# samyak0210/ViNet

Hardware: AMD Instinct MI355X
Metric: clips/sec training (32x224x384 bf16) (higher is better)
Workload: dtype bf16; 1 GPU; ViNet DHF1K training, 32x224x384 bf16, 192 clip(s)/GPU/step, kldiv + fused Adam, 1xMI355X; global_batch=192, local_batch=192, parallelism=dp1

## Files before the change

### include/vinet_hip.h

```cpp
#ifndef VINET_HIP_H
#define VINET_HIP_H

#include <stddef.h>
#include <stdint.h>

#ifdef __cplusplus
extern "C" {
#endif

#define VINET_ABI_VERSION 16

enum { VINET_F32 = 0, VINET_BF16 = 1,
       VINET_F32S = 2 };
enum { VINET_ACT_NONE = 0, VINET_ACT_RELU = 1, VINET_ACT_SIGMOID = 2 };
enum { VINET_CONV_GENERIC = 0, VINET_CONV_STEM = 1 };

typedef struct VinetTensor {
  void* ptr;
  int32_t B, T, H, W, C;
  int32_t ld;
  int64_t sB;
} VinetTensor;

typedef struct VinetAffine {
  const float* scale;
  const float* shift;
  int32_t relu;
} VinetAffine;

typedef struct VinetConvDesc {
  int32_t dtype;
  int32_t out_dtype;
  int32_t mode;
  VinetTensor x;
  VinetTensor y;
  int32_t oT, oH, oW;
  int32_t sT, sH, sW;
  int32_t omT, omH, omW, ooT, ooH, ooW;
  int32_t ntaps;
  const int32_t* taps;
  const void* w;
  int32_t Kp;
  VinetAffine pre;
  const float* out_scale;
  const float* out_shift;
  int32_t act;
  int32_t accumulate;
  float* stats;
  int32_t n_valid;
  float* splitk_ws;
  int64_t splitk_ws_bytes;
  int32_t tline;
  int32_t tpad;
  const void* bnb_z;
  int32_t bnb_ld;
  int64_t bnb_sB;
  VinetAffine bnb_fwd;
  const float* bnb_mean;
  const float* bnb_invstd;
  float* bnb_partials;
} VinetConvDesc;

int vinet_conv3d(const VinetConvDesc* desc, void* stream);
int64_t vinet_conv3d_splitk_bytes(const VinetConvDesc* desc);
int vinet_conv3d_fuses_dgrad_phases(const VinetConvDesc* desc);
int vinet_conv3d_bn_bwd_stats_rows(const VinetConvDesc* desc);
int vinet_conv3d_applies_pre_once(const VinetConvDesc* desc);
int vinet_conv3d_tile_m(const VinetConvDesc* desc);
int vinet_conv3d_stats_rows(const VinetConvDesc* desc);
int vinet_conv3d_kernel_name(const VinetConvDesc* desc, char* buf, int32_t n);

typedef struct VinetWgradDesc {
  int32_t dtype;
  int32_t mode;
  VinetTensor x;
  VinetTensor dy;
  int32_t sT, sH, sW;
  int32_t ntaps;
  const int32_t* taps;
  float* dw;
  int32_t Kp;
  VinetAffine pre;
  int32_t tline;
  int32_t tpad;
  const void* bnb_z;
  int32_t bnb_ld;
  int64_t bnb_sB;
  VinetAffine bnb_fwd;
  const float* bnb_mean;
  const float* bnb_invstd;
  const float* bnb_c1;
  const float* bnb_c2;
  int32_t max_cus;
} VinetWgradDesc;

int vinet_conv3d_wgrad(const VinetWgradDesc* desc, void* stream);
int vinet_conv3d_wgrad_fuses_bn_bwd(const VinetWgradDesc* desc);
int vinet_conv3d_wgrad_kernel_name(const VinetWgradDesc* desc, char* buf, int32_t n);

int vinet_pack_weights(const float* w, int32_t N, int32_t Cin, int32_t ntaps, int32_t transpose, int32_t stem,
                       int32_t dtype, void* out, void* stream);

int vinet_pack_weights_multi(const int64_t* table, int32_t njobs, int64_t total, int32_t dtype, void* stream);
int vinet_unpack_wgrad(float* dw, int32_t N, int32_t Cin, int32_t ntaps, int32_t stem, int32_t flags,
                       float* grad, void* stream);
int vinet_unpack_wgrad_multi(const int64_t* table, int32_t njobs, int64_t total, int32_t flags, void* stream);

int vinet_import_ncdhw(const float* src, int64_t sb, int64_t sc, int64_t st, int64_t sh, int64_t sw, int32_t C,
                       const VinetTensor* dst, int32_t dst_dtype, void* stream);
int vinet_import_ncdhw_pad(const float* src, int64_t sb, int64_t sc, int64_t st, int64_t sh, int64_t sw, int32_t C,
                           int32_t Hs, int32_t Ws, int32_t pad_top, int32_t pad_left, const VinetTensor* dst,
                           int32_t dst_dtype, void* stream);
int vinet_export_ncdhw(const VinetTensor* src, int32_t src_dtype, VinetAffine pre, float* dst, int64_t sb, int64_t sc,
                       int64_t st, int64_t sh, int64_t sw, int32_t accumulate, void* stream);
int vinet_copy_affine(const VinetTensor* src, int32_t src_dtype, VinetAffine pre, const VinetTensor* dst,
                      int32_t dst_dtype, int32_t accumulate, void* stream);

int vinet_bn_finalize(const float* partials, int32_t rows, int32_t C, int32_t ld, double count, const float* gamma,
                      const float* beta, float eps, float momentum, float* running_mean, float* running_var,
                      float* mean, float* invstd, float* scale, float* shift, void* stream);
int vinet_bn_partials_fold(const float* partials, int32_t rows, int32_t C, float* out, int32_t out_rows, void* stream);
int vinet_bn_fold(const float* gamma, const float* beta, const float* running_mean, const float* running_var,
                  const float* conv_bias , float eps, int32_t C, float* scale, float* shift,
                  float* invstd , void* stream);
int vinet_channel_stats(const VinetTensor* x, int32_t dtype, float* partials, void* stream);
int vinet_stats_rows(const VinetTensor* x);
int vinet_bn_bwd_reduce(const VinetTensor* dz, const VinetTensor* x_raw, int32_t dtype, VinetAffine fwd,
                        const float* mean, const float* invstd, float* partials, void* stream);
int vinet_bn_bwd_finalize(const float* partials, int32_t rows, int32_t C, int32_t ld, double count, const float* scale,
                          int32_t train, float* dgamma_acc, float* dbeta_acc, const float* invstd, float* c1, float* c2,
                          void* stream);
int vinet_bn_bwd_apply(const VinetTensor* dz, const VinetTensor* x_raw, int32_t dtype, VinetAffine fwd,
                       const float* mean, const float* invstd, const float* c1, const float* c2,
                       const VinetTensor* dx, void* stream);
int vinet_bn_bwd_apply_split(const VinetTensor* dz, const VinetTensor* x_raw, VinetAffine fwd, const float* mean,
                             const float* invstd, const float* c1, const float* c2, const VinetTensor* dx,
                             const VinetTensor* hi, const VinetTensor* lo, void* stream);
int vinet_act_bwd(const VinetTensor* dz, int32_t dz_dtype, const VinetTensor* z, int32_t z_dtype, int32_t act,
                  const VinetTensor* dy, int32_t dy_dtype, void* stream);
int vinet_channel_sum(const VinetTensor* x, int32_t dtype, float* workspace, int32_t Cout, float* out,
                      int32_t accumulate, void* stream);

typedef struct VinetPoolDesc {
  int32_t dtype;
  int32_t kT, kH, kW, sT, sH, sW, pT, pH, pW;
} VinetPoolDesc;
int vinet_maxpool3d(const VinetPoolDesc* d, const VinetTensor* x, VinetAffine pre, const VinetTensor* y,
                    uint8_t* argmax, void* stream);
int vinet_maxpool3d_bwd(const VinetPoolDesc* d, const VinetTensor* dy, const uint8_t* argmax, const VinetTensor* dx,
                        int32_t accumulate, void* stream);
int vinet_maxpool3d_kernel_name(const VinetPoolDesc* d, const VinetTensor* x, VinetAffine pre, const VinetTensor* y,
                                const uint8_t* argmax, char* buf, int32_t n);
int vinet_maxpool3d_bwd_kernel_name(const VinetPoolDesc* d, const VinetTensor* dy, const uint8_t* argmax,
                                    const VinetTensor* dx, char* buf, int32_t n);

int vinet_upsample2x(const VinetTensor* x, const VinetTensor* y, int32_t dtype, void* stream);
int vinet_upsample2x_bwd(const VinetTensor* dy, const VinetTensor* dx, int32_t dtype, int32_t accumulate, void* stream);
int vinet_upsample2x_bwd_relu(const VinetTensor* dy, const VinetTensor* dx, const VinetTensor* xf, int32_t dtype, void* stream);

int vinet_unfold1d(const VinetTensor* x, const VinetTensor* y, int32_t dtype, int32_t stride, int32_t pad, void* stream);

int vinet_loss_fwd(int32_t which, const float* s, const void* gt, int32_t gt_is_f64, int32_t B, int32_t n,
                   double* saved, float* loss, void* stream);
int vinet_loss_bwd(int32_t which, const float* s, const void* gt, int32_t gt_is_f64, int32_t B, int32_t n,
                   const double* saved, const float* gscale, float coeff, int32_t accumulate, float* ds, void* stream);

size_t vinet_auc_judd_workspace(int32_t B, int32_t n);
int vinet_auc_judd(const void* s, int32_t s_is_f64, const void* fix, int32_t fix_is_f64, int32_t B, int32_t n,
                   int32_t fp_offset, void* workspace, size_t workspace_bytes, double* score, int32_t* nfix,
                   int32_t* above, void* stream);

size_t vinet_auc_shuffled_workspace(int32_t B, int32_t n, int32_t nsplits, double step);
int vinet_auc_shuffled(const void* s, int32_t s_is_f64, const void* fix, int32_t fix_is_f64, const void* other,
                       int32_t other_kind, int64_t other_stride, int32_t B, int32_t n, int32_t nsplits, double step,
                       int64_t seed, const int64_t* frame_ids, const int32_t* samples, int32_t kmax, void* workspace,
                       size_t workspace_bytes, double* score, int32_t* nfix, int32_t* nother, int32_t* samples_out,
                       void* stream);

size_t vinet_auc_borji_workspace(int32_t B, int32_t n, int32_t nsplits, double step);
int vinet_auc_borji(const void* s, int32_t s_is_f64, const void* fix, int32_t fix_is_f64, int32_t B, int32_t n, int32_t nsplits,
                    double step, int64_t seed, const int64_t* frame_ids, const int32_t* samples, int32_t kmax, void* workspace,
                    size_t workspace_bytes, double* score, int32_t* nfix, int32_t* samples_out, void* stream);

int vinet_info_gain(const void* s, int32_t s_is_f64, const void* fix, int32_t fix_is_f64, const void* baseline,
                    int32_t baseline_is_f64, int64_t baseline_stride, int32_t B, int32_t n, double* score, int32_t* nfix,
                    void* stream);

size_t vinet_emd_workspace(int32_t B, int32_t R, int32_t C);
int vinet_emd(const void* s, int32_t s_is_f64, int32_t Hs, int32_t Ws, const void* gt, int32_t gt_is_f64, int32_t Hg, int32_t Wg,
              int32_t B, int32_t downsize, int32_t R, int32_t C, const double* w_gt_r, const double* w_gt_c, const double* w_s_r,
              const double* w_s_c, void* workspace, size_t workspace_bytes, double* score, int64_t* cost, int32_t* status,
              double* hist_out, void* stream);
int vinet_emd_hist(const double* P, const double* Q, int32_t B, int32_t R, int32_t C, void* workspace, size_t workspace_bytes,
                   double* score, int64_t* cost, int32_t* status, void* stream);

int vinet_adam_step(float* p, const float* g, float* m, float* v, int64_t n, float lr, float beta1, float beta2,
                    float eps, float bias_c1, float bias_c2, float grad_scale, void* stream);

int vinet_bilinear_fwd(const void* x1, const void* x2, int32_t dtype, const float* w, const float* bias, int32_t B,
                       int32_t C, int32_t I, int32_t J, int32_t O, void* out, void* stream);
int vinet_bilinear_bwd(const void* x1, const void* x2, const void* dout, int32_t dtype, const float* w, int32_t B,
                       int32_t C, int32_t I, int32_t J, int32_t O, void* dx1, void* dx2, float* dw, float* dbias,
                       void* stream);

typedef struct VinetTransformerDesc {
  int32_t dtype;
  int32_t B, S, E, H, F, L;
  int32_t train;
  float p, eps;
  uint64_t seed;
  int64_t* step;
  const float* pe;
  const void* const* params;
  void* const* grads;
  void* ws;
  int64_t ws_bytes;
  uint8_t* masks;
} VinetTransformerDesc;
int64_t vinet_transformer_workspace(const VinetTransformerDesc* desc);
int vinet_transformer_fwd(const VinetTransformerDesc* desc, const VinetTensor* x, const VinetTensor* y, void* stream);
int vinet_transformer_bwd(const VinetTransformerDesc* desc, const VinetTensor* dy, const VinetTensor* dx, void* stream);

typedef struct VinetTokenEncoderDesc {
  int32_t dtype;
  int32_t B, S, E, H, F, L;
  int32_t train;
  float p, eps;
  uint64_t seed;
  int64_t* step;
  const float* pe;
  const void* const* params;
  void* const* grads;
  void* ws;
  int64_t ws_bytes;
  uint8_t* masks;
} VinetTokenEncoderDesc;
int64_t vinet_token_encoder_workspace(const VinetTokenEncoderDesc* desc);
int vinet_token_encoder_fwd(const VinetTokenEncoderDesc* desc, const VinetTensor* x, const VinetTensor* y, void* stream);
int vinet_token_encoder_bwd(const VinetTokenEncoderDesc* desc, const VinetTensor* dy, const VinetTensor* dx, void* stream);
int vinet_token_split_fwd(const VinetTensor* x, int32_t dtype, int32_t n_audio, const VinetTensor* y, void* stream);
int vinet_token_split_bwd(const VinetTensor* dy, int32_t dtype, int32_t n_audio, const VinetTensor* dx, void* stream);

int vinet_resize_blur(const float* src, int32_t B, int32_t H, int32_t W, float* dst, int32_t oH, int32_t oW,
                      uint32_t* minmax, void* stream);
int vinet_minmax(const float* src, int32_t B, int64_t n, uint32_t* minmax, void* stream);
int vinet_normalize_u8(const float* src, const uint32_t* minmax, int32_t B, int64_t n, uint8_t* dst, void* stream);

int64_t vinet_frames_preprocess_ws_bytes(int32_t N, int32_t H, int32_t W, int32_t oH, int32_t oW);
int vinet_frames_preprocess(const uint8_t* src, int32_t N, int32_t H, int32_t W, float* dst, int32_t oH, int32_t oW,
                            const float* mean_std, void* ws, void* stream);
int vinet_audio_excerpt(const float* wav, int64_t n_samples, int64_t start, int64_t end, float* out, int32_t win, void* stream);
int64_t vinet_gt_preprocess_ws_bytes(int32_t N, int32_t oH, int32_t oW);
int vinet_gt_preprocess(const uint8_t* src, int32_t N, int32_t H, int32_t W, float* dst, int32_t oH, int32_t oW, void* ws,
                        void* stream);

int vinet_set_option(const char* name, int32_t value);
int vinet_split_bf16(const VinetTensor* src, VinetAffine pre, const VinetTensor* hi, const VinetTensor* lo, void* stream);
int vinet_fill_f32(float* p, int64_t n, float value, void* stream);
int vinet_debug_spin(int64_t cycles, void* stream);
int vinet_abi_version(void);
const char* vinet_last_error(void);

#ifdef __cplusplus
}
#endif
#endif
```

### vinet_amd/_lib.py

```python
import ctypes as C
import os

HERE = os.path.dirname(os.path.abspath(__file__))
LIB_PATH = os.environ.get("VINET_LIB") or os.path.join(HERE, "libvinet_hip.so")

F32, BF16 = 0, 1
F32S = 2
ACT_NONE, ACT_RELU, ACT_SIGMOID = 0, 1, 2
CONV_GENERIC, CONV_STEM = 0, 1
ABI_VERSION = 16


class CTensor(C.Structure):
    _fields_ = [("ptr", C.c_void_p), ("B", C.c_int32), ("T", C.c_int32), ("H", C.c_int32), ("W", C.c_int32),
                ("C", C.c_int32), ("ld", C.c_int32), ("sB", C.c_int64)]


class CAffine(C.Structure):
    _fields_ = [("scale", C.c_void_p), ("shift", C.c_void_p), ("relu", C.c_int32)]


class CConvDesc(C.Structure):
    _fields_ = [("dtype", C.c_int32), ("out_dtype", C.c_int32), ("mode", C.c_int32), ("x", CTensor), ("y", CTensor),
                ("oT", C.c_int32), ("oH", C.c_int32), ("oW", C.c_int32),
                ("sT", C.c_int32), ("sH", C.c_int32), ("sW", C.c_int32),
                ("omT", C.c_int32), ("omH", C.c_int32), ("omW", C.c_int32),
                ("ooT", C.c_int32), ("ooH", C.c_int32), ("ooW", C.c_int32),
                ("ntaps", C.c_int32), ("taps", C.c_void_p), ("w", C.c_void_p), ("Kp", C.c_int32),
                ("pre", CAffine), ("out_scale", C.c_void_p), ("out_shift", C.c_void_p),
                ("act", C.c_int32), ("accumulate", C.c_int32), ("stats", C.c_void_p), ("n_valid", C.c_int32),
                ("splitk_ws", C.c_void_p), ("splitk_ws_bytes", C.c_int64), ("tline", C.c_int32), ("tpad", C.c_int32),
                ("bnb_z", C.c_void_p), ("bnb_ld", C.c_int32), ("bnb_sB", C.c_int64), ("bnb_fwd", CAffine),
                ("bnb_mean", C.c_void_p), ("bnb_invstd", C.c_void_p), ("bnb_partials", C.c_void_p)]


class CWgradDesc(C.Structure):
    _fields_ = [("dtype", C.c_int32), ("mode", C.c_int32), ("x", CTensor), ("dy", CTensor),
                ("sT", C.c_int32), ("sH", C.c_int32), ("sW", C.c_int32),
                ("ntaps", C.c_int32), ("taps", C.c_void_p), ("dw", C.c_void_p), ("Kp", C.c_int32), ("pre", CAffine),
                ("tline", C.c_int32), ("tpad", C.c_int32),
                ("bnb_z", C.c_void_p), ("bnb_ld", C.c_int32), ("bnb_sB", C.c_int64), ("bnb_fwd", CAffine),
                ("bnb_mean", C.c_void_p), ("bnb_invstd", C.c_void_p), ("bnb_c1", C.c_void_p), ("bnb_c2", C.c_void_p),
                ("max_cus", C.c_int32)]


class CPoolDesc(C.Structure):
    _fields_ = [("dtype", C.c_int32)] + [(n, C.c_int32) for n in ("kT", "kH", "kW", "sT", "sH", "sW", "pT", "pH", "pW")]


class CTransformerDesc(C.Structure):
    _fields_ = [("dtype", C.c_int32), ("B", C.c_int32), ("S", C.c_int32), ("E", C.c_int32), ("H", C.c_int32), ("F", C.c_int32),
                ("L", C.c_int32), ("train", C.c_int32), ("p", C.c_float), ("eps", C.c_float), ("seed", C.c_uint64),
                ("step", C.c_void_p), ("pe", C.c_void_p), ("params", C.POINTER(C.c_void_p)), ("grads", C.POINTER(C.c_void_p)),
                ("ws", C.c_void_p), ("ws_bytes", C.c_int64), ("masks", C.c_void_p)]


class CTokenEncoderDesc(C.Structure):
    _fields_ = list(CTransformerDesc._fields_)


_vp, _i32, _i64, _f32, _f64 = C.c_void_p, C.c_int32, C.c_int64, C.c_float, C.c_double
_PT, _PC, _PW, _PP = C.POINTER(CTensor), C.POINTER(CConvDesc), C.POINTER(CWgradDesc), C.POINTER(CPoolDesc)
_PX = C.POINTER(CTransformerDesc)
_PK = C.POINTER(CTokenEncoderDesc)

SIGNATURES = {
    "vinet_conv3d": [_PC, _vp],
    "vinet_conv3d_tile_m": [_PC],
    "vinet_conv3d_stats_rows": [_PC],
    "vinet_conv3d_applies_pre_once": [_PC],
    "vinet_conv3d_splitk_bytes": [_PC],
    "vinet_conv3d_kernel_name": [_PC, C.c_char_p, _i32],
    "vinet_conv3d_wgrad": [_PW, _vp],
    "vinet_conv3d_wgrad_kernel_name": [_PW, C.c_char_p, _i32],
    "vinet_pack_weights": [_vp, _i32, _i32, _i32, _i32, _i32, _i32, _vp, _vp],
    "vinet_unpack_wgrad": [_vp, _i32, _i32, _i32, _i32, _i32, _vp, _vp],
    "vinet_import_ncdhw": [_vp, _i64, _i64, _i64, _i64, _i64, _i32, _PT, _i32, _vp],
    "vinet_import_ncdhw_pad": [_vp, _i64, _i64, _i64, _i64, _i64, _i32, _i32, _i32, _i32, _i32, _PT, _i32, _vp],
    "vinet_export_ncdhw": [_PT, _i32, CAffine, _vp, _i64, _i64, _i64, _i64, _i64, _i32, _vp],
    "vinet_copy_affine": [_PT, _i32, CAffine, _PT, _i32, _i32, _vp],
    "vinet_bn_finalize": [_vp, _i32, _i32, _i32, _f64, _vp, _vp, _f32, _f32, _vp, _vp, _vp, _vp, _vp, _vp, _vp],
    "vinet_bn_fold": [_vp, _vp, _vp, _vp, _vp, _f32, _i32, _vp, _vp, _vp, _vp],
    "vinet_channel_stats": [_PT, _i32, _vp, _vp],
    "vinet_stats_rows": [_PT],
    "vinet_bn_bwd_reduce": [_PT, _PT, _i32, CAffine, _vp, _vp, _vp, _vp],
    "vinet_conv3d_wgrad_fuses_bn_bwd": [_PW],
    "vinet_conv3d_fuses_dgrad_phases": [_PC],
    "vinet_conv3d_bn_bwd_stats_rows": [_PC],
    "vinet_bn_partials_fold": [_vp, _i32, _i32, _vp, _i32, _vp],
    "vinet_bn_bwd_finalize": [_vp, _i32, _i32, _i32, _f64, _vp, _i32, _vp, _vp, _vp, _vp, _vp, _vp],
    "vinet_bn_bwd_apply": [_PT, _PT, _i32, CAffine, _vp, _vp, _vp, _vp, _PT, _vp],
    "vinet_bn_bwd_apply_split": [_PT, _PT, CAffine, _vp, _vp, _vp, _vp, _PT, _PT, _PT, _vp],
    "vinet_act_bwd": [_PT, _i32, _PT, _i32, _i32, _PT, _i32, _vp],
    "vinet_channel_sum": [_PT, _i32, _vp, _i32, _vp, _i32, _vp],
    "vinet_maxpool3d": [_PP, _PT, CAffine, _PT, _vp, _vp],
    "vinet_maxpool3d_bwd": [_PP, _PT, _vp, _PT, _i32, _vp],
    "vinet_maxpool3d_kernel_name": [_PP, _PT, CAffine, _PT, _vp, C.c_char_p, _i32],
    "vinet_maxpool3d_bwd_kernel_name": [_PP, _PT, _vp, _PT, C.c_char_p, _i32],
    "vinet_upsample2x": [_PT, _PT, _i32, _vp],
    "vinet_unfold1d": [_PT, _PT, _i32, _i32, _i32, _vp],
    "vinet_upsample2x_bwd": [_PT, _PT, _i32, _i32, _vp],
    "vinet_upsample2x_bwd_relu": [_PT, _PT, _PT, _i32, _vp],
    "vinet_loss_fwd": [_i32, _vp, _vp, _i32, _i32, _i32, _vp, _vp, _vp],
    "vinet_loss_bwd": [_i32, _vp, _vp, _i32, _i32, _i32, _vp, _vp, _f32, _i32, _vp, _vp],
    "vinet_auc_judd_workspace": [_i32, _i32],
    "vinet_auc_judd": [_vp, _i32, _vp, _i32, _i32, _i32, _i32, _vp, C.c_size_t, _vp, _vp, _vp, _vp],
    "vinet_auc_shuffled_workspace": [_i32, _i32, _i32, _f64],
    "vinet_auc_shuffled": [_vp, _i32, _vp, _i32, _vp, _i32, _i64, _i32, _i32, _i32, _f64, _i64, _vp, _vp, _i32, _vp, C.c_size_t,
                           _vp, _vp, _vp, _vp, _vp],
    "vinet_auc_borji_workspace": [_i32, _i32, _i32, _f64],
    "vinet_auc_borji": [_vp, _i32, _vp, _i32, _i32, _i32, _i32, _f64, _i64, _vp, _vp, _i32, _vp, C.c_size_t, _vp, _vp, _vp, _vp],
    "vinet_info_gain": [_vp, _i32, _vp, _i32, _vp, _i32, _i64, _i32, _i32, _vp, _vp, _vp],
    "vinet_emd_workspace": [_i32, _i32, _i32],
    "vinet_emd": [_vp, _i32, _i32, _i32, _vp, _i32, _i32, _i32, _i32, _i32, _i32, _i32, _vp, _vp, _vp, _vp, _vp, C.c_size_t, _vp, _vp, _vp, _vp,
                  _vp],
    "vinet_emd_hist": [_vp, _vp, _i32, _i32, _i32, _vp, C.c_size_t, _vp, _vp, _vp, _vp],
    "vinet_adam_step": [_vp, _vp, _vp, _vp, _i64, _f32, _f32, _f32, _f32, _f32, _f32, _f32, _vp],
    "vinet_bilinear_fwd": [_vp, _vp, _i32, _vp, _vp, _i32, _i32, _i32, _i32, _i32, _vp, _vp],
    "vinet_bilinear_bwd": [_vp, _vp, _vp, _i32, _vp, _i32, _i32, _i32, _i32, _i32, _vp, _vp, _vp, _vp, _vp],
    "vinet_transformer_workspace": [_PX],
    "vinet_transformer_fwd": [_PX, _PT, _PT, _vp],
    "vinet_transformer_bwd": [_PX, _PT, _PT, _vp],
    "vinet_token_encoder_workspace": [_PK],
    "vinet_token_encoder_fwd": [_PK, _PT, _PT, _vp],
    "vinet_token_encoder_bwd": [_PK, _PT, _PT, _vp],
    "vinet_token_split_fwd": [_PT, _i32, _i32, _PT, _vp],
    "vinet_token_split_bwd": [_PT, _i32, _i32, _PT, _vp],
    "vinet_resize_blur": [_vp, _i32, _i32, _i32, _vp, _i32, _i32, _vp, _vp],
    "vinet_minmax": [_vp, _i32, _i64, _vp, _vp],
    "vinet_normalize_u8": [_vp, _vp, _i32, _i64, _vp, _vp],
    "vinet_frames_preprocess_ws_bytes": [_i32, _i32, _i32, _i32, _i32],
    "vinet_frames_preprocess": [_vp, _i32, _i32, _i32, _vp, _i32, _i32, C.POINTER(C.c_float), _vp, _vp],
    "vinet_audio_excerpt": [_vp, _i64, _i64, _i64, _vp, _i32, _vp],
    "vinet_gt_preprocess_ws_bytes": [_i32, _i32, _i32],
    "vinet_gt_preprocess": [_vp, _i32, _i32, _i32, _vp, _i32, _i32, _vp, _vp],
    "vinet_set_option": [C.c_char_p, _i32],
    "vinet_pack_weights_multi": [_vp, _i32, _i64, _i32, _vp],
    "vinet_unpack_wgrad_multi": [_vp, _i32, _i64, _i32, _vp],
    "vinet_fill_f32": [_vp, _i64, _f32, _vp],
    "vinet_split_bf16": [_PT, CAffine, _PT, _PT, _vp],
    "vinet_debug_spin": [_i64, _vp],
    "vinet_abi_version": [],
    "vinet_last_error": [],
}
_RESTYPE = {"vinet_last_error": C.c_char_p, "vinet_conv3d_splitk_bytes": C.c_int64, "vinet_frames_preprocess_ws_bytes": C.c_int64,
            "vinet_gt_preprocess_ws_bytes": C.c_int64, "vinet_auc_judd_workspace": C.c_size_t, "vinet_auc_shuffled_workspace": C.c_size_t, "vinet_auc_borji_workspace": C.c_size_t,
            "vinet_emd_workspace": C.c_size_t,
            "vinet_transformer_workspace": C.c_int64, "vinet_token_encoder_workspace": C.c_int64}

_LIB = None
_TEST_DOUBLE = None


class VinetLibraryError(RuntimeError):
    pass


def load(path=LIB_PATH):
    global _LIB
    if _LIB is not None:
        return _LIB
    if not os.path.exists(path):
        raise VinetLibraryError(
            "libvinet_hip.so is missing (%s). Build it with `python -m vinet_amd.build` "
            "(hipcc --offload-arch=gfx950); there is no CPU fallback." % path)
    import torch
    lib = C.CDLL(path)
    for name, argtypes in SIGNATURES.items():
        try:
            fn = getattr(lib, name)
        except AttributeError:
            raise VinetLibraryError("libvinet_hip.so does not export %s" % name)
        fn.argtypes = argtypes
        fn.restype = _RESTYPE.get(name, C.c_int)
    if lib.vinet_abi_version() != ABI_VERSION:
        raise VinetLibraryError("libvinet_hip.so ABI %d != expected %d" % (lib.vinet_abi_version(), ABI_VERSION))
    _LIB = lib
    return lib


LIB_OPTIONS = {}


def set_option(name, value):
    lib = get()
    rc = lib.vinet_set_option(name.encode() if isinstance(name, str) else name, int(value))
    if rc != 0:
        msg = lib.vinet_last_error()
        raise VinetLibraryError("set_option(%s): %s" % (name, msg.decode() if isinstance(msg, bytes) else msg))
    LIB_OPTIONS[name if isinstance(name, str) else name.decode()] = int(value)


def get():
    if _TEST_DOUBLE is not None:
        return _TEST_DOUBLE
    return load()


def is_test_double():
    return _TEST_DOUBLE is not None


def _install_test_double(obj):
    global _TEST_DOUBLE
    _TEST_DOUBLE = obj


def check(rc, what=""):
    if rc != 0:
        lib = get()
        msg = lib.vinet_last_error()
        if isinstance(msg, bytes):
            msg = msg.decode()
        raise RuntimeError("libvinet_hip %s failed (rc=%d): %s" % (what, rc, msg))
```

### vinet_amd/build.py

```python
import os
import subprocess
import sys
from concurrent.futures import ThreadPoolExecutor

HERE = os.path.dirname(os.path.abspath(__file__))
ROOT = os.path.dirname(HERE)
CSRC = os.path.join(HERE, "csrc")
OBJ = os.path.join(CSRC, "obj")
LIB = os.path.join(HERE, "libvinet_hip.so")
SOURCES = ["conv_api.hip", "conv_bf16.hip", "conv_bnb.hip", "conv_f32.hip", "conv_wgrad.hip", "wgrad_dma.hip", "wgrad_pp.hip", "wgrad_ts.hip", "conv_ts.hip", "wgrad_hs.hip", "wgrad_rs.hip", "wgrad_tf.hip", "conv_hs.hip", "layout.hip", "bn.hip", "pool.hip", "resample.hip", "loss_adam.hip", "metrics.hip", "emd.hip", "postproc.hip", "preproc.hip", "transformer.hip", "token_encoder.hip"]
import glob
HEADERS = sorted(glob.glob(os.path.join(CSRC, "*.h"))) + sorted(glob.glob(os.path.join(ROOT, "include", "*.h")))
FLAGS = ["--offload-arch=gfx950", "-O3", "-std=c++17", "-fPIC", "-I" + os.path.join(ROOT, "include"), "-I" + CSRC,
         "-Wno-unused-result", "-ffp-contract=off"]


GUARDED = {"conv_bf16.hip": ("conv_pw_kernel",), "pool.hip": ("maxpool_bwd",), "conv_bnb.hip": ()}
RESOURCES = os.path.join(CSRC, "obj", "kernel_resources.json")


def _parse_resources(text):
    import re
    out, cur = {}, None
    keys = {"VGPRs": "vgpr", "AGPRs": "agpr", "TotalSGPRs": "sgpr", "ScratchSize [bytes/lane]": "scratch", "VGPRs Spill": "vgpr_spill",
            "SGPRs Spill": "sgpr_spill", "Occupancy [waves/SIMD]": "occupancy"}
    for line in text.splitlines():
        m = re.search(r"remark:\s+Function Name: (\S+)", line)
        if m:
            cur = out.setdefault(m.group(1), {})
            continue
        m = re.search(r"remark:\s+([A-Za-z \[\]/]+): (\d+)", line)
        if m and cur is not None and m.group(1).strip() in keys:
            cur[keys[m.group(1).strip()]] = int(m.group(2))
    return out


def check_guarded(src, text):
    res = _parse_resources(text)
    bad = [(k, v) for k, v in res.items() if any(g in k for g in GUARDED.get(src, ())) and v.get("vgpr_spill", 0) > 0]
    if bad:
        raise RuntimeError("vector-register spills in kernels whose inline asm owns in-flight registers (%s): %s" % (src, bad))
    return res


def _hipcc():
    for c in (os.environ.get("HIPCC"), "/opt/rocm/bin/hipcc", "hipcc"):
        if c and (os.path.isabs(c) and os.path.exists(c) or not os.path.isabs(c)):
            return c
    raise RuntimeError("hipcc not found")


def _stale(target, deps):
    if not os.path.exists(target):
        return True
    t = os.path.getmtime(target)
    return any(os.path.getmtime(d) > t for d in deps)


def build_variant(tag, extra_flags, verbose=True):
    global OBJ, LIB, FLAGS
    save = (OBJ, LIB, FLAGS)
    OBJ, LIB, FLAGS = os.path.join(CSRC, "obj_" + tag), os.path.join(HERE, "libvinet_hip_%s.so" % tag), FLAGS + list(extra_flags)
    try:
        return build(force=False, verbose=verbose)
    finally:
        OBJ, LIB, FLAGS = save


def build(force=False, verbose=True):
    os.makedirs(OBJ, exist_ok=True)
    hipcc = _hipcc()
    hdrs = [h if os.path.isabs(h) else os.path.join(CSRC, h) for h in HEADERS]
    jobs = []
    for src in SOURCES:
        s = os.path.join(CSRC, src)
        o = os.path.join(OBJ, src.replace(".hip", ".o"))
        if force or _stale(o, [s] + hdrs):
            jobs.append((s, o))

    def compile_one(job):
        s, o = job
        guarded = os.path.basename(s) in GUARDED
        cmd = [hipcc] + FLAGS + (["-Rpass-analysis=kernel-resource-usage"] if guarded else []) + ["-c", s, "-o", o]
        r = subprocess.run(cmd, capture_output=True, text=True)
        out = r.stdout + r.stderr
        if guarded and r.returncode == 0:
            try:
                res = check_guarded(os.path.basename(s), out)
            except RuntimeError:
                os.remove(o)
                raise
            out = "\n".join(l for l in out.splitlines() if "kernel-resource-usage" not in l and not l.startswith("   ") )
            return s, r.returncode, out, res
        return s, r.returncode, out, None

    if jobs:
        if verbose:
            print("[vinet_amd.build] compiling %d file(s) for gfx950 ..." % len(jobs), flush=True)
        with ThreadPoolExecutor(max_workers=min(len(jobs), os.cpu_count() or 4)) as ex:
            resources, failed = {}, None
            for s, rc, out, res in ex.map(compile_one, jobs):
                if rc != 0:
                    failed = failed or RuntimeError("hipcc failed on %s:\n%s" % (s, out))
                    continue
                if res is not None:
                    resources[os.path.basename(s)] = res
                if verbose and out.strip():
                    print(out)
        if resources:
            import json
            try:
                allres = json.load(open(RESOURCES)) if os.path.exists(RESOURCES) else {}
            except ValueError:
                allres = {}
            allres.update(resources)
            with open(RESOURCES, "w") as f:
                json.dump(allres, f, indent=1, sort_keys=True)
        if failed is not None:
            raise failed
    objs = [os.path.join(OBJ, s.replace(".hip", ".o")) for s in SOURCES]
    if force or jobs or _stale(LIB, objs):
        cmd = [hipcc, "--offload-arch=gfx950", "-shared", "-fPIC", "-o", LIB] + objs
        r = subprocess.run(cmd, capture_output=True, text=True)
        if r.returncode != 0:
            raise RuntimeError("link failed:\n" + r.stdout + r.stderr)
        if verbose:
            print("[vinet_amd.build] linked", LIB, flush=True)
        try:
            audit_packed_fp32(LIB, verbose)
        except RuntimeError:
            os.remove(LIB)
            raise
    return LIB


def audit_packed_fp32(lib, verbose=True):
    import importlib.util
    spec = importlib.util.spec_from_file_location("vinet_isa_audit", os.path.join(ROOT, "tools", "isa_audit.py"))
    ia = importlib.util.module_from_spec(spec)
    spec.loader.exec_module(ia)
    if not os.path.exists(ia.OBJDUMP):
        print("[vinet_amd.build] WARNING: %s missing -- the packed-fp32 erratum audit of %s did NOT run" % (ia.OBJDUMP, lib), file=sys.stderr, flush=True)
        return None
    hits = ia.packed_fp32_high_half_reads(lib)
    if hits:
        raise RuntimeError("packed fp32 instructions with op_sel:[x,1] (MI355X erratum form) in %s: %s -- build those kernels with VN_NO_PK_F32" % (lib, hits))
    if verbose:
        print("[vinet_amd.build] packed-fp32 erratum audit: clean", flush=True)
    return hits


if __name__ == "__main__":
    build(force="--force" in sys.argv)
```

### vinet_amd/csrc/bn.hip

```cpp
#include "elementwise.h"

__global__ void bn_finalize_kernel(const float* __restrict__ partials, int rows, int C, int ld, double count,
                                   const float* gamma, const float* beta, float eps, float momentum,
                                   float* running_mean, float* running_var, float* mean_o, float* invstd_o,
                                   float* scale_o, float* shift_o) {
  const int c = blockIdx.x;
  double s = 0.0, q = 0.0;
  for (int r = threadIdx.x; r < rows; r += blockDim.x) {
    s += (double)partials[((long)r * 2 + 0) * ld + c];
    q += (double)partials[((long)r * 2 + 1) * ld + c];
  }
  __shared__ double red[2][4];
  s = wave_sum_d(s); q = wave_sum_d(q);
  if ((threadIdx.x & 63) == 0) { red[0][threadIdx.x >> 6] = s; red[1][threadIdx.x >> 6] = q; }
  __syncthreads();
  if (threadIdx.x == 0) {
    s = red[0][0] + red[0][1] + red[0][2] + red[0][3];
    q = red[1][0] + red[1][1] + red[1][2] + red[1][3];
    const double mean = s / count;
    double var = q / count - mean * mean;
    if (var < 0.0) var = 0.0;
    const double invstd = 1.0 / sqrt(var + (double)eps);
    const float g = gamma ? gamma[c] : 1.f, b = beta ? beta[c] : 0.f;
    const float sc = (float)(g * invstd);
    if (mean_o) mean_o[c] = (float)mean;
    if (invstd_o) invstd_o[c] = (float)invstd;
    scale_o[c] = sc;
    shift_o[c] = b - (float)mean * sc;
    if (running_mean) running_mean[c] = (1.f - momentum) * running_mean[c] + momentum * (float)mean;
    if (running_var) {
      const double unbiased = count > 1.0 ? var * count / (count - 1.0) : var;
      running_var[c] = (1.f - momentum) * running_var[c] + momentum * (float)unbiased;
    }
  }
}

extern "C" int vinet_bn_finalize(const float* partials, int32_t rows, int32_t C, int32_t ld, double count, const float* gamma,
                                 const float* beta, float eps, float momentum, float* running_mean, float* running_var,
                                 float* mean, float* invstd, float* scale, float* shift, void* stream) {
  VN_CHECK_ARG(partials && rows > 0 && C > 0 && (ld == 0 || ld >= C) && count > 0 && scale && shift, "bn_finalize: bad arguments");
  hipLaunchKernelGGL(bn_finalize_kernel, dim3(C), dim3(256), 0, (hipStream_t)stream, partials, rows, C, ld ? ld : C, count, gamma,
                     beta, eps, momentum, running_mean, running_var, mean, invstd, scale, shift);
  return vn_launch_status("bn_finalize");
}

__global__ __launch_bounds__(256) void bn_partials_fold_kernel(const float* __restrict__ partials, int rows, int C, int per,
                                                               float* __restrict__ out) {
  const int c = blockIdx.y * 64 + (threadIdx.x & 63), rl = threadIdx.x >> 6;
  const int r0 = blockIdx.x * per;
  int r1 = r0 + per; if (r1 > rows) r1 = rows;
  double s = 0.0, q = 0.0;
  if (c < C) {
    int r = r0 + rl;
    for (; r + 28 < r1; r += 32) {
      float a[8], b[8];
#pragma unroll
      for (int u = 0; u < 8; ++u) {
        a[u] = partials[((long)(r + 4 * u) * 2 + 0) * C + c];
        b[u] = partials[((long)(r + 4 * u) * 2 + 1) * C + c];
      }
#pragma unroll
      for (int u = 0; u < 8; ++u) { s += (double)a[u]; q += (double)b[u]; }
    }
    for (; r < r1; r += 4) {
      s += (double)partials[((long)r * 2 + 0) * C + c];
      q += (double)partials[((long)r * 2 + 1) * C + c];
    }
  }
  __shared__ double red[2][4][64];
  red[0][rl][threadIdx.x & 63] = s; red[1][rl][threadIdx.x & 63] = q;
  __syncthreads();
  if (rl == 0 && c < C) {
    const int l = threadIdx.x;
    out[((long)blockIdx.x * 2 + 0) * C + c] = (float)(red[0][0][l] + red[0][1][l] + red[0][2][l] + red[0][3][l]);
    out[((long)blockIdx.x * 2 + 1) * C + c] = (float)(red[1][0][l] + red[1][1][l] + red[1][2][l] + red[1][3][l]);
  }
}

extern "C" int vinet_bn_partials_fold(const float* partials, int32_t rows, int32_t C, float* out, int32_t out_rows, void* stream) {
  VN_CHECK_ARG(partials && out && rows > 0 && C > 0 && out_rows > 0 && out_rows <= rows, "bn_partials_fold: bad arguments");
  const int per = (rows + out_rows - 1) / out_rows;
  VN_CHECK_ARG((long)(out_rows - 1) * per < rows, "bn_partials_fold: out_rows=%d leaves empty chunks for rows=%d", out_rows, rows);
  hipLaunchKernelGGL(bn_partials_fold_kernel, dim3(out_rows, (C + 63) / 64), dim3(256), 0, (hipStream_t)stream, partials, rows, C, per, out);
  return vn_launch_status("bn_partials_fold");
}

__global__ void bn_fold_kernel(const float* gamma, const float* beta, const float* rm, const float* rv,
                               const float* conv_bias, float eps, int C, float* scale, float* shift, float* invstd) {
  const int c = blockIdx.x * blockDim.x + threadIdx.x;
  if (c >= C) return;
  const float is = 1.f / sqrtf(rv[c] + eps);
  const float sc = (gamma ? gamma[c] : 1.f) * is;
  scale[c] = sc;
  shift[c] = (beta ? beta[c] : 0.f) + ((conv_bias ? conv_bias[c] : 0.f) - rm[c]) * sc;
  if (invstd) invstd[c] = is;
}

extern "C" int vinet_bn_fold(const float* gamma, const float* beta, const float* running_mean,
                             const float* running_var, const float* conv_bias, float eps, int32_t C, float* scale,
                             float* shift, float* invstd, void* stream) {
  VN_CHECK_ARG(running_mean && running_var && scale && shift && C > 0, "bn_fold: bad arguments");
  hipLaunchKernelGGL(bn_fold_kernel, dim3((C + 255) / 256), dim3(256), 0, (hipStream_t)stream, gamma, beta,
                     running_mean, running_var, conv_bias, eps, C, scale, shift, invstd);
  return vn_launch_status("bn_fold");
}


template <typename T, int MODE>
__global__ __launch_bounds__(256) VN_NO_PK_F32 void channel_reduce8_kernel(TView x, TView dz, Affine fwd, const float* mean,
                                                              const float* invstd, long nvox, long vb,
                                                              float* __restrict__ partials) {
  const int G = x.C / 8;
  const int Gb = G < 256 ? G : 256;
  const int R = 256 / Gb;
  const int r = threadIdx.x / Gb;
  const int g0 = threadIdx.x % Gb;
  __shared__ float red[256 * 16];
  constexpr int U = 4;
  const long v0 = vb ? (long)blockIdx.x * vb : (long)blockIdx.x * R * U;
  long v1 = vb ? v0 + vb : nvox; if (v1 > nvox) v1 = nvox;
  const long vstep = vb ? (long)R * U : (long)gridDim.x * R * U;
  for (int g = g0; g < G; g += Gb) {
    float s[8], p[8], mu[8], is[8], sc[8], sh[8];
#pragma unroll
    for (int e = 0; e < 8; ++e) { s[e] = 0.f; p[e] = 0.f; mu[e] = 0.f; is[e] = 1.f; sc[e] = 1.f; sh[e] = 0.f; }
    if (r < R) {
      if (MODE == 1) {
#pragma unroll
        for (int e = 0; e < 8; ++e) { mu[e] = mean[g * 8 + e]; is[e] = invstd[g * 8 + e]; }
        if (fwd.relu) {
#pragma unroll
          for (int e = 0; e < 8; ++e) { sc[e] = fwd.scale ? fwd.scale[g * 8 + e] : 1.f; sh[e] = fwd.shift ? fwd.shift[g * 8 + e] : 0.f; }
        }
      }
      for (long vq = v0 + r; vq < v1; vq += vstep) {
        float xv[U][8], gv[U][8];
        bool ok[U];
#pragma unroll
        for (int u = 0; u < U; ++u) {
          const long v = vq + (long)u * R;
          ok[u] = v < v1;
          if (ok[u]) {
            if (MODE == 1) {
              ld8_nt<T>((const T*)x.p + vox_lin(x, v) + g * 8, xv[u]);
              ld8_nt<T>((const T*)dz.p + vox_lin(dz, v) + g * 8, gv[u]);
            } else {
              ld8<T>((const T*)x.p + vox_lin(x, v) + g * 8, xv[u]);
            }
          }
        }
#pragma unroll
        for (int u = 0; u < U; ++u) {
          if (!ok[u]) continue;
// ... 326 lines not shown
  long v1 = v0 + vb; if (v1 > nvox) v1 = nvox;
  for (int g = g0; g < G; g += Gb) {
    float A[8], Bc[8], D[8], sh[8];
#pragma unroll
    for (int e = 0; e < 8; ++e) {
      const int c = g * 8 + e;
      const float sc = fwd.scale[c], k = sc * invstd[c] * c2[c];
      A[e] = sc; Bc[e] = -k; D[e] = fmaf(k, mean[c], -sc * c1[c]);
      sh[e] = fwd.shift[c];
    }
    constexpr int U = 4;
    for (long vq = v0 + r; vq < v1; vq += (long)R * U) {
      float xv[U][8], gv[U][8];
      bool ok[U];
#pragma unroll
      for (int u = 0; u < U; ++u) {
        const long v = vq + (long)u * R;
        ok[u] = v < v1;
        if (ok[u]) {
          ld8_nt<T>((const T*)x.p + vox_lin(x, v) + g * 8, xv[u]);
          ld8<T>((const T*)dz.p + vox_lin(dz, v) + g * 8, gv[u]);
        }
      }
#pragma unroll
      for (int u = 0; u < U; ++u) {
        if (!ok[u]) continue;
        float o[8];
#pragma unroll
        for (int e = 0; e < 8; ++e) {
          float gg = gv[u][e];
          if (fwd.relu && !(fmaf(xv[u][e], A[e], sh[e]) > 0.f)) gg = 0.f;
          o[e] = fmaf(A[e], gg, fmaf(Bc[e], xv[u][e], D[e]));
        }
        st8_nt<T>((T*)dx.p + vox_lin(dx, vq + (long)u * R) + g * 8, o);
        if constexpr (SPLIT) {
          uint32_t h[4], l[4];
#pragma unroll
          for (int e = 0; e < 4; ++e) {
            h[e] = pack2bf(o[2 * e], o[2 * e + 1]);
            l[e] = pack2bf(o[2 * e] - __uint_as_float(h[e] << 16), o[2 * e + 1] - __uint_as_float(h[e] & 0xffff0000u));
          }
          st16_nt((bf16_t*)hi.p + vox_lin(hi, vq + (long)u * R) + g * 8, make_uint4(h[0], h[1], h[2], h[3]));
          st16_nt((bf16_t*)lo.p + vox_lin(lo, vq + (long)u * R) + g * 8, make_uint4(l[0], l[1], l[2], l[3]));
        }
      }
    }
  }
}

template <int U, int WPE>
__global__ __launch_bounds__(256, WPE) void bn_bwd_apply8_bf16_kernel(TView dz, TView x, Affine fwd, const float* mean, const float* invstd,
                                                                 const float* c1, const float* c2, TView dx, long nvox, long vb) {
  const int G = x.C / 8;
  const int Gb = G < 256 ? G : 256;
  const int R = 256 / Gb;
  const int r = threadIdx.x / Gb;
  const int g0 = threadIdx.x % Gb;
  if (r >= R) return;
  const long v0 = (long)blockIdx.x * vb;
  long v1 = v0 + vb; if (v1 > nvox) v1 = nvox;
  const bool relu = fwd.relu != 0;
  for (int g = g0; g < G; g += Gb) {
    float A[8], Bc[8], D[8], sh[8];
#pragma unroll
    for (int e = 0; e < 8; ++e) {
      const int c = g * 8 + e;
      const float sc = fwd.scale[c], k = sc * invstd[c] * c2[c];
      A[e] = sc; Bc[e] = -k; D[e] = fmaf(k, mean[c], -sc * c1[c]);
      sh[e] = fwd.shift[c];
    }
    for (long vq = v0 + r; vq < v1; vq += (long)R * U) {
      uint4 xr[U], gr[U];
#pragma unroll
      for (int u = 0; u < U; ++u) {
        const long v = vq + (long)u * R;
        const long vc = v < v1 ? v : vq;
        xr[u] = ld16_nt((const bf16_t*)x.p + vox_lin(x, vc) + g * 8);
        gr[u] = *(const uint4*)((const bf16_t*)dz.p + vox_lin(dz, vc) + g * 8);
      }
#pragma unroll
      for (int u = 0; u < U; ++u) {
        if (vq + (long)u * R >= v1) continue;
        const uint32_t xw[4] = {xr[u].x, xr[u].y, xr[u].z, xr[u].w}, gw[4] = {gr[u].x, gr[u].y, gr[u].z, gr[u].w};
        uint32_t ow[4];
#pragma unroll
        for (int h = 0; h < 4; ++h) {
          float o2[2];
#pragma unroll
          for (int k2 = 0; k2 < 2; ++k2) {
            const int e = 2 * h + k2;
            const float xv = __uint_as_float(k2 ? (xw[h] & 0xffff0000u) : (xw[h] << 16));
            float gg = __uint_as_float(k2 ? (gw[h] & 0xffff0000u) : (gw[h] << 16));
            if (relu && !(fmaf(xv, A[e], sh[e]) > 0.f)) gg = 0.f;
            o2[k2] = fmaf(A[e], gg, fmaf(Bc[e], xv, D[e]));
          }
          ow[h] = pack2bf(o2[0], o2[1]);
        }
        st16_nt((bf16_t*)dx.p + vox_lin(dx, vq + (long)u * R) + g * 8, make_uint4(ow[0], ow[1], ow[2], ow[3]));
      }
    }
  }
}

extern "C" int vinet_bn_bwd_apply(const VinetTensor* dz, const VinetTensor* x_raw, int32_t dtype, VinetAffine fwd,
                                  const float* mean, const float* invstd, const float* c1, const float* c2,
                                  const VinetTensor* dx, void* stream) {
  VN_CHECK_ARG(dz && x_raw && dx && fwd.scale && fwd.shift && mean && invstd && c1 && c2, "bn_bwd_apply: null argument");
  VN_CHECK_ARG(quad_ok(*dz, esize(dtype)) && quad_ok(*x_raw, esize(dtype)) && quad_ok(*dx, esize(dtype)) &&
                   same_dims(*dz, *x_raw) && same_dims(*dz, *dx), "bn_bwd_apply: bad views");
  if (oct_ok(*dz) && oct_ok(*x_raw) && oct_ok(*dx)) {
    const long nvox = view_voxels(*dz);
    const int G = dz->C / 8, R = 256 / (G < 256 ? G : 256);
    long vb = R * 16;
    while ((nvox + vb - 1) / vb > 16384) vb *= 2;
    if (g_vinet_opt_bn_lean && dtype == VINET_BF16) {
#ifdef VINET_EXPERIMENTS
      if (g_vinet_opt_bn_lean == 2)
        hipLaunchKernelGGL((bn_bwd_apply8_bf16_kernel<2, 6>), dim3((unsigned)((nvox + vb - 1) / vb)), dim3(256), 0, (hipStream_t)stream,
                           make_view(*dz), make_view(*x_raw), make_affine(fwd), mean, invstd, c1, c2, make_view(*dx), nvox, vb);
      else
#endif
        hipLaunchKernelGGL((bn_bwd_apply8_bf16_kernel<4, 4>), dim3((unsigned)((nvox + vb - 1) / vb)), dim3(256), 0, (hipStream_t)stream,
                           make_view(*dz), make_view(*x_raw), make_affine(fwd), mean, invstd, c1, c2, make_view(*dx), nvox, vb);
      return vn_launch_status("bn_bwd_apply8_bf16");
    }
    DISPATCH_T(dtype, T, hipLaunchKernelGGL((bn_bwd_apply8_kernel<T, false>), dim3((unsigned)((nvox + vb - 1) / vb)), dim3(256), 0,
                                            (hipStream_t)stream, make_view(*dz), make_view(*x_raw), make_affine(fwd), mean,
                                            invstd, c1, c2, make_view(*dx), make_view(*dx), make_view(*dx), nvox, vb);)
    return vn_launch_status("bn_bwd_apply8");
  }
  const long total = view_voxels(*dz) * (dz->C / 4);
  DISPATCH_T(dtype, T, hipLaunchKernelGGL(bn_bwd_apply_kernel<T>, dim3(ew_grid(total)), dim3(256), 0,
                                          (hipStream_t)stream, make_view(*dz), make_view(*x_raw), make_affine(fwd), mean,
                                          invstd, c1, c2, make_view(*dx), total);)
  return vn_launch_status("bn_bwd_apply");
}

extern "C" int vinet_bn_bwd_apply_split(const VinetTensor* dz, const VinetTensor* x_raw, VinetAffine fwd, const float* mean,
                                        const float* invstd, const float* c1, const float* c2, const VinetTensor* dx,
                                        const VinetTensor* hi, const VinetTensor* lo, void* stream) {
  VN_CHECK_ARG(dz && x_raw && dx && hi && lo && fwd.scale && fwd.shift && mean && invstd && c1 && c2, "bn_bwd_apply_split: null argument");
  VN_CHECK_ARG(oct_ok(*dz) && oct_ok(*x_raw) && oct_ok(*dx) && oct_ok(*hi) && oct_ok(*lo) && same_dims(*dz, *x_raw) && same_dims(*dz, *dx) &&
                   same_dims(*dz, *hi) && same_dims(*dz, *lo) && quad_ok(*dz, 4) && quad_ok(*x_raw, 4) && quad_ok(*dx, 4) && quad_ok(*hi, 2) &&
                   quad_ok(*lo, 2), "bn_bwd_apply_split: bad views (fp32 tensors, bf16 planes, C a multiple of 8)");
  const long nvox = view_voxels(*dz);
  const int G = dz->C / 8, R = 256 / (G < 256 ? G : 256);
  long vb = R * 16;
  while ((nvox + vb - 1) / vb > 16384) vb *= 2;
  hipLaunchKernelGGL((bn_bwd_apply8_kernel<float, true>), dim3((unsigned)((nvox + vb - 1) / vb)), dim3(256), 0, (hipStream_t)stream,
                     make_view(*dz), make_view(*x_raw), make_affine(fwd), mean, invstd, c1, c2, make_view(*dx), make_view(*hi), make_view(*lo), nvox, vb);
  return vn_launch_status("bn_bwd_apply8<split>");
}

template <typename TG, typename TZ, typename TO>
__global__ void act_bwd_kernel(TView dz, TView z, int act, TView dy, long total) {
  const long i = (long)blockIdx.x * blockDim.x + threadIdx.x;
  if (i >= total) return;
  const uint32_t vox_u = fdiv((uint32_t)i, z.dQ);
  const int q = (int)((uint32_t)i - vox_u * (uint32_t)(z.C / 4));
  const long vox = (long)vox_u;
  const float4 zv = ldq<TZ>((const TZ*)z.p + vox_lin(z, vox) + q * 4);
  float4 g = ldq<TG>((const TG*)dz.p + vox_lin(dz, vox) + q * 4);
  if (act == VINET_ACT_RELU) {
    if (!(zv.x > 0.f)) g.x = 0.f;
    if (!(zv.y > 0.f)) g.y = 0.f;
    if (!(zv.z > 0.f)) g.z = 0.f;
    if (!(zv.w > 0.f)) g.w = 0.f;
  } else if (act == VINET_ACT_SIGMOID) {
    g.x *= zv.x * (1.f - zv.x); g.y *= zv.y * (1.f - zv.y); g.z *= zv.z * (1.f - zv.z); g.w *= zv.w * (1.f - zv.w);
  }
  stq<TO>((TO*)dy.p + vox_lin(dy, vox) + q * 4, g);
}

extern "C" int vinet_act_bwd(const VinetTensor* dz, int32_t dz_dtype, const VinetTensor* z, int32_t z_dtype,
                             int32_t act, const VinetTensor* dy, int32_t dy_dtype, void* stream) {
  VN_CHECK_ARG(dz && z && dy && quad_ok(*dz, esize(dz_dtype)) && quad_ok(*z, esize(z_dtype)) &&
                   quad_ok(*dy, esize(dy_dtype)) && same_dims(*dz, *z) && same_dims(*dz, *dy), "act_bwd: bad views");
  const long total = view_voxels(*z) * (z->C / 4);
  const dim3 g(ew_grid(total)), blk(256);
  hipStream_t s = (hipStream_t)stream;
  const TView a = make_view(*dz), b = make_view(*z), c = make_view(*dy);
#define ACT_CASE(D1, T1, D2, T2, D3, T3) \
  if (dz_dtype == D1 && z_dtype == D2 && dy_dtype == D3) { hipLaunchKernelGGL((act_bwd_kernel<T1, T2, T3>), g, blk, 0, s, a, b, act, c, total); return vn_launch_status("act_bwd"); }
  ACT_CASE(VINET_F32, float, VINET_F32, float, VINET_F32, float)
  ACT_CASE(VINET_BF16, bf16_t, VINET_BF16, bf16_t, VINET_BF16, bf16_t)
  ACT_CASE(VINET_F32, float, VINET_F32, float, VINET_BF16, bf16_t)
  ACT_CASE(VINET_F32, float, VINET_BF16, bf16_t, VINET_BF16, bf16_t)
  ACT_CASE(VINET_BF16, bf16_t, VINET_F32, float, VINET_BF16, bf16_t)
#undef ACT_CASE
  vinet_set_error("act_bwd: unsupported dtype combination %d/%d/%d", dz_dtype, z_dtype, dy_dtype);
  return -1;
}

__global__ __launch_bounds__(256) void channel_sum_finalize_kernel(const float* __restrict__ partials, int rows, int C,
                                                                   int Cout, float* out, int accumulate) {
  const int j = blockIdx.x;
  double s = 0.0;
  const int per = C / Cout;
  for (int e = threadIdx.x; e < rows * per; e += blockDim.x) {
    const int r = e / per, c = j + (e % per) * Cout;
    s += (double)partials[((long)r * 2) * C + c];
  }
  __shared__ double red[4];
  s = wave_sum_d(s);
  if ((threadIdx.x & 63) == 0) red[threadIdx.x >> 6] = s;
  __syncthreads();
  if (threadIdx.x == 0) {
    s = red[0] + red[1] + red[2] + red[3];
    if (accumulate) atomicAdd(out + j, (float)s);
    else out[j] = (float)s;
  }
}

extern "C" int vinet_channel_sum(const VinetTensor* x, int32_t dtype, float* workspace, int32_t Cout, float* out,
                                 int32_t accumulate, void* stream) {
  VN_CHECK_ARG(x && workspace && out && Cout > 0 && quad_ok(*x, esize(dtype)) && x->C % Cout == 0, "channel_sum: bad arguments");
  VinetAffine none = {nullptr, nullptr, 0};
  int rc = launch_channel_reduce<0>(x, nullptr, dtype, none, nullptr, nullptr, workspace, stream);
  if (rc) return rc;
  hipLaunchKernelGGL(channel_sum_finalize_kernel, dim3(Cout), dim3(256), 0, (hipStream_t)stream, workspace,
                     stats_rows_for(view_voxels(*x)), x->C, Cout, out, accumulate);
  return vn_launch_status("channel_sum");
}
```

### vinet_amd/csrc/pool.hip

```cpp
#include "elementwise.h"

struct PoolP { int kT, kH, kW, sT, sH, sW, pT, pH, pW; FastDiv dsT, dsH, dsW; };
static inline PoolP make_poolp(const VinetPoolDesc* d) {
  PoolP p = {d->kT, d->kH, d->kW, d->sT, d->sH, d->sW, d->pT, d->pH, d->pW, make_fastdiv((uint32_t)d->sT), make_fastdiv((uint32_t)d->sH), make_fastdiv((uint32_t)d->sW)};
  return p;
}

template <typename T> VN_DEV float pool_round(float v) { return v; }
template <> VN_DEV float pool_round<bf16_t>(float v) { return bf2f(f2bf(v)); }
template <typename T> VN_DEV float4 pool_pre4(float4 v, const Affine& pre, int c) {
  v = affine4(v, pre, c);
  if (pre.scale) { v.x = pool_round<T>(v.x); v.y = pool_round<T>(v.y); v.z = pool_round<T>(v.z); v.w = pool_round<T>(v.w); }
  return v;
}
template <typename T> VN_DEV float pool_pre(float f, float sc, float sh, const Affine& pre) {
  float v = fmaf(f, sc, sh);
  if (pre.relu) v = fmaxf(v, 0.f);
  if (pre.scale) v = pool_round<T>(v);
  return v;
}
VN_DEV void pool_column(const TView& v, uint32_t col, int& b, int& h, int& w) {
  const uint32_t r1 = fdiv(col, v.dW);
  w = (int)(col - r1 * (uint32_t)v.W);
  const uint32_t r2 = fdiv(r1, v.dH);
  h = (int)(r1 - r2 * (uint32_t)v.H);
  b = (int)r2;
}

template <typename T>
__global__ void maxpool_fwd_kernel(PoolP p, TView x, Affine pre, TView y, uint8_t* __restrict__ argmax, long total) {
  const long i = (long)blockIdx.x * blockDim.x + threadIdx.x;
  if (i >= total) return;
  const uint32_t vox_u = fdiv((uint32_t)i, y.dQ);
  const int q = (int)((uint32_t)i - vox_u * (uint32_t)(y.C / 4));
  const long vox = (long)vox_u;
  int b, to, ho, wo;
  decode_vox(y, vox, b, to, ho, wo);
  float best[4] = {-INFINITY, -INFINITY, -INFINITY, -INFINITY};
  int bi[4] = {0, 0, 0, 0};
  for (int kt = 0; kt < p.kT; ++kt) {
    const int t = to * p.sT - p.pT + kt;
    if ((unsigned)t >= (unsigned)x.T) continue;
    for (int kh = 0; kh < p.kH; ++kh) {
      const int h = ho * p.sH - p.pH + kh;
      if ((unsigned)h >= (unsigned)x.H) continue;
      for (int kw = 0; kw < p.kW; ++kw) {
        const int w = wo * p.sW - p.pW + kw;
        if ((unsigned)w >= (unsigned)x.W) continue;
        const float4 v = pool_pre4<T>(ldq<T>((const T*)x.p + vox_off(x, b, t, h, w) + q * 4), pre, q * 4);
        const int tap = (kt * p.kH + kh) * p.kW + kw;
        const float f[4] = {v.x, v.y, v.z, v.w};
#pragma unroll
        for (int e = 0; e < 4; ++e)
          if (f[e] > best[e] || (f[e] != f[e] && best[e] == best[e])) { best[e] = f[e]; bi[e] = tap; }
      }
    }
  }
  stq<T>((T*)y.p + vox_off(y, b, to, ho, wo) + q * 4, make_float4(best[0], best[1], best[2], best[3]));
  if (argmax) *(uint32_t*)(argmax + vox * y.C + q * 4) = (uint32_t)bi[0] | ((uint32_t)bi[1] << 8) | ((uint32_t)bi[2] << 16) | ((uint32_t)bi[3] << 24);
}

template <typename T>
__global__ void maxpool_tslide_kernel(PoolP p, TView x, Affine pre, TView y, uint8_t* __restrict__ argmax, long total) {
  const long i = (long)blockIdx.x * blockDim.x + threadIdx.x;
  if (i >= total) return;
  const uint32_t col = fdiv((uint32_t)i, y.dQ);
  const int q = (int)((uint32_t)i - col * (uint32_t)(y.C / 4));
  int b, ho, wo;
  pool_column(y, col, b, ho, wo);
  float pm[3][4];
  int pa[3][4];
  const int khw = p.kH * p.kW;
  for (int tp = 0; tp <= x.T; ++tp) {
    const int slot = tp % 3;
    if (tp < x.T) {
      float best[4] = {-INFINITY, -INFINITY, -INFINITY, -INFINITY};
      int bi[4] = {0, 0, 0, 0};
      for (int kh = 0; kh < p.kH; ++kh) {
        const int h = ho * p.sH - p.pH + kh;
        if ((unsigned)h >= (unsigned)x.H) continue;
        for (int kw = 0; kw < p.kW; ++kw) {
          const int w = wo * p.sW - p.pW + kw;
          if ((unsigned)w >= (unsigned)x.W) continue;
          float4 v = pool_pre4<T>(ldq<T>((const T*)x.p + vox_off(x, b, tp, h, w) + q * 4), pre, q * 4);
          if (pre.scale) { v.x = pool_round<T>(v.x); v.y = pool_round<T>(v.y); v.z = pool_round<T>(v.z); v.w = pool_round<T>(v.w); }
          const float f[4] = {v.x, v.y, v.z, v.w};
#pragma unroll
          for (int e = 0; e < 4; ++e)
            if (f[e] > best[e] || (f[e] != f[e] && best[e] == best[e])) { best[e] = f[e]; bi[e] = kh * p.kW + kw; }
        }
      }
#pragma unroll
      for (int e = 0; e < 4; ++e) { pm[slot][e] = best[e]; pa[slot][e] = bi[e]; }
    }
    const int to = tp - 1;
    if (to < 0) continue;
    float o[4];
    int oi[4];
#pragma unroll
    for (int e = 0; e < 4; ++e) { o[e] = -INFINITY; oi[e] = 0; }
#pragma unroll
    for (int kt = 0; kt < 3; ++kt) {
      const int t = to - 1 + kt;
      if (t < 0 || t >= x.T) continue;
      const int sl = t % 3;
#pragma unroll
      for (int e = 0; e < 4; ++e)
        if (pm[sl][e] > o[e] || (pm[sl][e] != pm[sl][e] && o[e] == o[e])) { o[e] = pm[sl][e]; oi[e] = kt * khw + pa[sl][e]; }
    }
    stq<T>((T*)y.p + vox_off(y, b, to, ho, wo) + q * 4, make_float4(o[0], o[1], o[2], o[3]));
    if (argmax) {
      const long ovox = (((long)b * y.T + to) * y.H + ho) * y.W + wo;
      *(uint32_t*)(argmax + ovox * y.C + q * 4) = (uint32_t)oi[0] | ((uint32_t)oi[1] << 8) | ((uint32_t)oi[2] << 16) | ((uint32_t)oi[3] << 24);
    }
  }
}

VN_DEV void affine8(float* v, const Affine& a, int c) {
  if (a.scale) {
#pragma unroll
    for (int e = 0; e < 8; ++e) v[e] = fmaf(v[e], a.scale[c + e], a.shift[c + e]);
  }
  if (a.relu) {
#pragma unroll
    for (int e = 0; e < 8; ++e) v[e] = fmaxf(v[e], 0.f);
  }
}

template <typename T>
__global__ __launch_bounds__(256) void maxpool_fwd8_kernel(PoolP p, TView x, Affine pre, TView y, uint8_t* __restrict__ argmax, long total) {
  const long i = (long)blockIdx.x * blockDim.x + threadIdx.x;
  if (i >= total) return;
  const int G = y.C >> 3;
  const uint32_t vox_u = (uint32_t)(i / G);
  const int g = (int)(i - (long)vox_u * G);
  int b, to, ho, wo;
  decode_vox(y, (long)vox_u, b, to, ho, wo);
  float sc[8], sh[8];
#pragma unroll
  for (int e = 0; e < 8; ++e) { sc[e] = pre.scale ? pre.scale[g * 8 + e] : 1.f; sh[e] = pre.scale ? pre.shift[g * 8 + e] : 0.f; }
  float best[8];
  unsigned long long bi = 0;
#pragma unroll
  for (int e = 0; e < 8; ++e) best[e] = -INFINITY;
  for (int kt = 0; kt < p.kT; ++kt) {
    const int t = to * p.sT - p.pT + kt;
    if ((unsigned)t >= (unsigned)x.T) continue;
    for (int kh = 0; kh < p.kH; ++kh) {
      const int h = ho * p.sH - p.pH + kh;
      if ((unsigned)h >= (unsigned)x.H) continue;
      for (int kw = 0; kw < p.kW; ++kw) {
        const int w = wo * p.sW - p.pW + kw;
        if ((unsigned)w >= (unsigned)x.W) continue;
// ... 203 lines not shown
  int b, to, ho, wo;
  decode_vox(y, (long)vox_u, b, to, ho, wo);
  f32x2_v sc2[4], sh2[4];
  const bool aff = pre.scale != nullptr;
#pragma unroll
  for (int e = 0; e < 4; ++e) {
    sc2[e] = aff ? (f32x2_v){pre.scale[g * 8 + 2 * e], pre.scale[g * 8 + 2 * e + 1]} : (f32x2_v){1.f, 1.f};
    sh2[e] = aff ? (f32x2_v){pre.shift[g * 8 + 2 * e], pre.shift[g * 8 + 2 * e + 1]} : (f32x2_v){0.f, 0.f};
  }
  uint32_t best[8];
#pragma unroll
  for (int e = 0; e < 8; ++e) best[e] = 0;
  const uint32_t last = (uint32_t)(p.kT * p.kH * p.kW - 1);
  for (int kt = 0; kt < p.kT; ++kt) {
    const int t = to * p.sT - p.pT + kt;
    if ((unsigned)t >= (unsigned)x.T) continue;
    for (int kh = 0; kh < p.kH; ++kh) {
      const int h = ho * p.sH - p.pH + kh;
      if ((unsigned)h >= (unsigned)x.H) continue;
      for (int kw = 0; kw < p.kW; ++kw) {
        const int w = wo * p.sW - p.pW + kw;
        if ((unsigned)w >= (unsigned)x.W) continue;
        const uint4 q = *(const uint4*)((const bf16_t*)x.p + vox_off(x, b, t, h, w) + g * 8);
        uint32_t w4[4] = {q.x, q.y, q.z, q.w};
        const uint32_t ck = last - (uint32_t)((kt * p.kH + kh) * p.kW + kw);
#pragma unroll
        for (int e = 0; e < 4; ++e) {
          if (aff) {
            if (pre.relu) w4[e] = pre_relu_pair(w4[e], sc2[e], sh2[e]);
            else w4[e] = pack2bf(fmaf(__uint_as_float(w4[e] << 16), sc2[e].x, sh2[e].x), fmaf(__uint_as_float(w4[e] & 0xffff0000u), sc2[e].y, sh2[e].y));
          } else if (pre.relu) {
            asm("v_pk_max_i16 %0, %1, 0" : "=v"(w4[e]) : "v"(w4[e]));
          }
          const uint32_t c = pool_code2(w4[e]);
          const uint32_t klo = (c << 16) | ck, khi = (c & 0xffff0000u) | ck;
          best[2 * e] = best[2 * e] > klo ? best[2 * e] : klo;
          best[2 * e + 1] = best[2 * e + 1] > khi ? best[2 * e + 1] : khi;
        }
      }
    }
  }
  uint32_t ov[4];
  unsigned long long bi = 0;
#pragma unroll
  for (int e = 0; e < 8; ++e) {
    const uint32_t k = best[e];
    if (e & 1) ov[e >> 1] |= k & 0xffff0000u; else ov[e >> 1] = k >> 16;
    bi |= (unsigned long long)(last - (k & 0xffu)) << (8 * e);
  }
  uint4 o;
  o.x = pool_decode2(ov[0]); o.y = pool_decode2(ov[1]); o.z = pool_decode2(ov[2]); o.w = pool_decode2(ov[3]);
  *(uint4*)((bf16_t*)y.p + vox_off(y, b, to, ho, wo) + g * 8) = o;
  if (argmax) *(unsigned long long*)(argmax + (long)vox_u * y.C + g * 8) = bi;
}

__global__ __launch_bounds__(512) void maxpool_k3s1_pk_kernel(TView x, Affine pre, TView y, uint8_t* __restrict__ argmax,
                                                              int tilesH, int tilesW) {
  __shared__ __attribute__((aligned(16))) uint16_t P[2][100][64];
  __shared__ __attribute__((aligned(16))) float S[2][64];
  const int tid = threadIdx.x;
  const int oct = tid & 7, pos = tid >> 3;
  const int ph = pos >> 3, pw = pos & 7;
  int bid = blockIdx.x;
  const int ncg = (x.C + 63) >> 6;
  const int cg = bid % ncg; bid /= ncg;
  const int tw = bid % tilesW; bid /= tilesW;
  const int th = bid % tilesH; bid /= tilesH;
  const int b = bid;
  const int h0 = th * 8, w0 = tw * 8, c0 = cg * 64 + oct * 8;
  const int ho = h0 + ph, wo = w0 + pw;
  const bool out_ok = ho < y.H && wo < y.W && c0 < x.C;
  const bool aff = pre.scale != nullptr;
  if (tid < 64) {
    const bool ok = aff && cg * 64 + tid < x.C;
    S[0][tid] = ok ? pre.scale[cg * 64 + tid] : 1.f;
    S[1][tid] = ok ? pre.shift[cg * 64 + tid] : 0.f;
  }
  __syncthreads();
  uint32_t m_a[8], m_b[8], m_c[8];
#pragma unroll
  for (int e = 0; e < 8; ++e) { m_a[e] = 0; m_b[e] = 0; m_c[e] = 0; }
  const int T_ = x.T;
  for (int tp = 0; tp <= T_; ++tp) {
    uint16_t (*buf)[64] = P[tp & 1];
    if (tp < T_) {
      for (int it = tid; it < 800; it += 512) {
        const int hp = it >> 3;
        const int hh = h0 - 1 + hp / 10, ww = w0 - 1 + hp % 10;
        if (cg * 64 + oct * 8 >= x.C) continue;
        uint4 q = make_uint4(0, 0, 0, 0);
        if ((unsigned)hh < (unsigned)x.H && (unsigned)ww < (unsigned)x.W) {
          q = *(const uint4*)((const bf16_t*)x.p + vox_off(x, b, tp, hh, ww) + cg * 64 + oct * 8);
          if (aff) {
            const float2* sp = (const float2*)&S[0][oct * 8];
            const float2* hp2 = (const float2*)&S[1][oct * 8];
            uint32_t* w4 = (uint32_t*)&q;
#pragma unroll
            for (int e = 0; e < 4; ++e) {
              const float2 s2 = sp[e], h2 = hp2[e];
              if (pre.relu) w4[e] = pre_relu_pair(w4[e], (f32x2_v){s2.x, s2.y}, (f32x2_v){h2.x, h2.y});
              else w4[e] = pack2bf(fmaf(__uint_as_float(w4[e] << 16), s2.x, h2.x), fmaf(__uint_as_float(w4[e] & 0xffff0000u), s2.y, h2.y));
            }
          } else if (pre.relu) {
            uint32_t* w4 = (uint32_t*)&q;
#pragma unroll
            for (int e = 0; e < 4; ++e) asm("v_pk_max_i16 %0, %1, 0" : "=v"(w4[e]) : "v"(w4[e]));
          }
          q.x = pool_code2(q.x); q.y = pool_code2(q.y); q.z = pool_code2(q.z); q.w = pool_code2(q.w);
        }
        *(uint4*)&buf[hp][oct * 8] = q;
      }
    }
    __syncthreads();
#pragma unroll
    for (int e = 0; e < 8; ++e) { m_a[e] = m_b[e]; m_b[e] = m_c[e]; m_c[e] = 0; }
    if (tp < T_) {
#pragma unroll
      for (int kh = 0; kh < 3; ++kh)
#pragma unroll
        for (int kw = 0; kw < 3; ++kw) {
          const uint4 q = *(const uint4*)&buf[(ph + kh) * 10 + pw + kw][oct * 8];
          const uint32_t ck = 8u - (uint32_t)(kh * 3 + kw);
          const uint32_t w4[4] = {q.x, q.y, q.z, q.w};
#pragma unroll
          for (int e = 0; e < 4; ++e) {
            const uint32_t klo = (w4[e] << 16) | ck, khi = (w4[e] & 0xffff0000u) | ck;
            m_c[2 * e] = m_c[2 * e] > klo ? m_c[2 * e] : klo;
            m_c[2 * e + 1] = m_c[2 * e + 1] > khi ? m_c[2 * e + 1] : khi;
          }
        }
    }
    const int to = tp - 1;
    if (to < 0 || !out_ok) continue;
    uint32_t ov[4];
    unsigned long long oi = 0;
    const bool va = to >= 1, vc = to + 1 < T_;
#pragma unroll
    for (int e = 0; e < 8; ++e) {
      const uint32_t ka = va ? m_a[e] + 18u : 0u, kb = m_b[e] + 9u, kc = vc ? m_c[e] : 0u;
      uint32_t k = ka > kb ? ka : kb;
      k = k > kc ? k : kc;
      if (e & 1) ov[e >> 1] |= k & 0xffff0000u; else ov[e >> 1] = k >> 16;
      oi |= (unsigned long long)(26u - (k & 0xffu)) << (8 * e);
    }
    uint4 o;
    o.x = pool_decode2(ov[0]); o.y = pool_decode2(ov[1]); o.z = pool_decode2(ov[2]); o.w = pool_decode2(ov[3]);
    *(uint4*)((bf16_t*)y.p + vox_off(y, b, to, ho, wo) + c0) = o;
    if (argmax) {
      const long ovox = (((long)b * y.T + to) * y.H + ho) * y.W + wo;
      *(unsigned long long*)(argmax + ovox * y.C + c0) = oi;
    }
  }
}

#define POOL_ADD_IF_X(g, word, BYTE, code, v, exec0)                                                                                  \
  asm volatile("v_cmpx_eq_u32_sdwa vcc, %1, %2 src0_sel:BYTE_" #BYTE " src1_sel:DWORD\n\tv_add_f32_e32 %0, %0, %3\n\ts_mov_b64 exec, %4" \
               : "+v"(g) : "v"(word), "s"(code), "v"(v), "s"(exec0) : "vcc")
#define POOL_ADD_IF(g, word, BYTE, code, v) POOL_ADD_IF_X(g, word, BYTE, code, v, exec0)
#define POOL_ADD_IF8(g, lo, hi, e, code, v, ex)                                           \
  do {                                                                                      \
    const uint32_t w_ = (e) < 4 ? (lo) : (hi);                                              \
    switch ((e) & 3) {                                                                      \
      case 0: POOL_ADD_IF_X(g, w_, 0, code, v, ex); break;                                  \
      case 1: POOL_ADD_IF_X(g, w_, 1, code, v, ex); break;                                  \
      case 2: POOL_ADD_IF_X(g, w_, 2, code, v, ex); break;                                  \
      default: POOL_ADD_IF_X(g, w_, 3, code, v, ex); break;                                 \
    }                                                                                       \
  } while (0)

template <typename T>
__global__ void maxpool_bwd_kernel(PoolP p, TView dy, const uint8_t* __restrict__ argmax, TView dx, int accumulate,
                                   long total) {
  const long i = (long)blockIdx.x * blockDim.x + threadIdx.x;
  if (i >= total) return;
  const uint32_t vox_u = fdiv((uint32_t)i, dx.dQ);
  const int q = (int)((uint32_t)i - vox_u * (uint32_t)(dx.C / 4));
  const long vox = (long)vox_u;
  int b, t, h, w;
  decode_vox(dx, vox, b, t, h, w);
  float g[4] = {0, 0, 0, 0};
  const int to1 = min((int)fdiv((uint32_t)(t + p.pT), p.dsT), dy.T - 1), ho1 = min((int)fdiv((uint32_t)(h + p.pH), p.dsH), dy.H - 1),
            wo1 = min((int)fdiv((uint32_t)(w + p.pW), p.dsW), dy.W - 1);
  const int to0 = (int)fdiv((uint32_t)max(0, t + p.pT - p.kT + p.sT), p.dsT), ho0 = (int)fdiv((uint32_t)max(0, h + p.pH - p.kH + p.sH), p.dsH),
            wo0 = (int)fdiv((uint32_t)max(0, w + p.pW - p.kW + p.sW), p.dsW);
  for (int to = to0; to <= to1; ++to) {
    const int kt = t + p.pT - to * p.sT;
    if (kt < 0 || kt >= p.kT) continue;
    for (int ho = ho0; ho <= ho1; ++ho) {
      const int kh = h + p.pH - ho * p.sH;
      if (kh < 0 || kh >= p.kH) continue;
      for (int wo = wo0; wo <= wo1; ++wo) {
        const int kw = w + p.pW - wo * p.sW;
        if (kw < 0 || kw >= p.kW) continue;
        const uint32_t tap = (uint32_t)((kt * p.kH + kh) * p.kW + kw);
        const long ovox = (((long)b * dy.T + to) * dy.H + ho) * dy.W + wo;
        const uint32_t am = *(const uint32_t*)(argmax + ovox * dy.C + q * 4);
        const uint32_t xr = am ^ (tap * 0x01010101u);
        if (!((xr - 0x01010101u) & ~xr & 0x80808080u)) continue;
        const float4 d = ldq<T>((const T*)dy.p + vox_off(dy, b, to, ho, wo) + q * 4);
        if ((xr & 0xffu) == 0) g[0] += d.x;
        if ((xr & 0xff00u) == 0) g[1] += d.y;
        if ((xr & 0xff0000u) == 0) g[2] += d.z;
        if ((xr & 0xff000000u) == 0) g[3] += d.w;
      }
    }
  }
  T* dst = (T*)dx.p + vox_off(dx, b, t, h, w) + q * 4;
  if (accumulate) { const float4 o = ldq<T>(dst); g[0] += o.x; g[1] += o.y; g[2] += o.z; g[3] += o.w; }
  stq<T>(dst, make_float4(g[0], g[1], g[2], g[3]));
}

template <typename T>
__global__ __launch_bounds__(256) void maxpool_bwd_k3s1_kernel(TView dy, const uint8_t* __restrict__ argmax, TView dx,
                                                               int accumulate, long total) {
  const long i = (long)blockIdx.x * blockDim.x + threadIdx.x;
  if (i >= total) return;
  const int G = dx.C >> 3;
  const uint32_t vox_u = (uint32_t)(i / G);
  const int g = (int)(i - (long)vox_u * G);
  int b, t, h, w;
  decode_vox(dx, (long)vox_u, b, t, h, w);
  const int T_ = dx.T, H = dx.H, W = dx.W;
  const long am_c = (long)vox_u * dx.C + g * 8;
  const long dy_c = vox_off(dy, b, t, h, w) + g * 8;
  unsigned long long am[27];
#pragma unroll
  for (int kt = 0; kt < 3; ++kt)
#pragma unroll
    for (int kh = 0; kh < 3; ++kh)
#pragma unroll
      for (int kw = 0; kw < 3; ++kw) {
        const int dt = 1 - kt, dh = 1 - kh, dw = 1 - kw;
        const bool ok = (unsigned)(t + dt) < (unsigned)T_ && (unsigned)(h + dh) < (unsigned)H && (unsigned)(w + dw) < (unsigned)W;
        const long d = ((long)(dt * H + dh) * W + dw) * (long)dx.C;
        am[(kt * 3 + kh) * 3 + kw] = ok ? *(const unsigned long long*)(argmax + am_c + d) : ~0ull;
      }
  float gr[8] = {0, 0, 0, 0, 0, 0, 0, 0};
#pragma unroll
  for (int kt = 0; kt < 3; ++kt)
#pragma unroll
    for (int kh = 0; kh < 3; ++kh)
#pragma unroll
      for (int kw = 0; kw < 3; ++kw) {
        const int tap = (kt * 3 + kh) * 3 + kw;
        const unsigned long long xr = am[tap] ^ (0x0101010101010101ull * (unsigned long long)tap);
        if (!((xr - 0x0101010101010101ull) & ~xr & 0x8080808080808080ull)) continue;
        const int dt = 1 - kt, dh = 1 - kh, dw = 1 - kw;
        const T* src = (const T*)dy.p + dy_c + ((long)(dt * H + dh) * W + dw) * (long)dy.ld;
        const float4 d0 = ldq<T>(src), d1 = ldq<T>(src + 4);
        const float dv[8] = {d0.x, d0.y, d0.z, d0.w, d1.x, d1.y, d1.z, d1.w};
#pragma unroll
        for (int e = 0; e < 8; ++e)
          if (((xr >> (8 * e)) & 0xffull) == 0) gr[e] += dv[e];
      }
  T* dst = (T*)dx.p + vox_off(dx, b, t, h, w) + g * 8;
  if (accumulate) {
    const float4 o0 = ldq<T>(dst), o1 = ldq<T>(dst + 4);
    gr[0] += o0.x; gr[1] += o0.y; gr[2] += o0.z; gr[3] += o0.w; gr[4] += o1.x; gr[5] += o1.y; gr[6] += o1.z; gr[7] += o1.w;
  }
  stq<T>(dst, make_float4(gr[0], gr[1], gr[2], gr[3]));
  stq<T>(dst + 4, make_float4(gr[4], gr[5], gr[6], gr[7]));
}

template <typename T>
__global__ __launch_bounds__(256) void maxpool_bwd8_kernel(PoolP p, TView dy, const uint8_t* __restrict__ argmax, TView dx, int accumulate,
                                                           long total) {
  const long i = (long)blockIdx.x * blockDim.x + threadIdx.x;
  if (i >= total) return;
  const int G = dx.C >> 3;
  const uint32_t vox_u = (uint32_t)(i / G);
  const int g = (int)(i - (long)vox_u * G);
  int b, t, h, w;
  decode_vox(dx, (long)vox_u, b, t, h, w);
  float gr[8] = {0, 0, 0, 0, 0, 0, 0, 0};
  const int to1 = min((int)fdiv((uint32_t)(t + p.pT), p.dsT), dy.T - 1), ho1 = min((int)fdiv((uint32_t)(h + p.pH), p.dsH), dy.H - 1),
            wo1 = min((int)fdiv((uint32_t)(w + p.pW), p.dsW), dy.W - 1);
  const int to0 = (int)fdiv((uint32_t)max(0, t + p.pT - p.kT + p.sT), p.dsT), ho0 = (int)fdiv((uint32_t)max(0, h + p.pH - p.kH + p.sH), p.dsH),
            wo0 = (int)fdiv((uint32_t)max(0, w + p.pW - p.kW + p.sW), p.dsW);
  for (int to = to0; to <= to1; ++to) {
    const int kt = t + p.pT - to * p.sT;
    if (kt < 0 || kt >= p.kT) continue;
    for (int ho = ho0; ho <= ho1; ++ho) {
      const int kh = h + p.pH - ho * p.sH;
      if (kh < 0 || kh >= p.kH) continue;
      for (int wo = wo0; wo <= wo1; ++wo) {
        const int kw = w + p.pW - wo * p.sW;
        if (kw < 0 || kw >= p.kW) continue;
        const unsigned long long tap = (unsigned long long)((kt * p.kH + kh) * p.kW + kw);
        const long ovox = (((long)b * dy.T + to) * dy.H + ho) * dy.W + wo;
        const unsigned long long am = *(const unsigned long long*)(argmax + ovox * dy.C + g * 8);
        const unsigned long long xr = am ^ (tap * 0x0101010101010101ull);
        if (!((xr - 0x0101010101010101ull) & ~xr & 0x8080808080808080ull)) continue;
        float dv[8];
        ld8<T>((const T*)dy.p + vox_off(dy, b, to, ho, wo) + g * 8, dv);
#pragma unroll
        for (int e = 0; e < 8; ++e)
          if (((xr >> (8 * e)) & 0xffull) == 0) gr[e] += dv[e];
      }
    }
  }
  T* dst = (T*)dx.p + vox_off(dx, b, t, h, w) + g * 8;
  if (accumulate) {
    float o[8];
    ld8<T>(dst, o);
#pragma unroll
    for (int e = 0; e < 8; ++e) gr[e] += o[e];
  }
  st8<T>(dst, gr);
}

template <typename T>
__global__ __launch_bounds__(256) void maxpool_bwd_k133s2_kernel(TView dy, const uint8_t* __restrict__ argmax, TView dx, int accumulate,
                                                                 int HB, int WB, long total) {
  const long i = (long)blockIdx.x * blockDim.x + threadIdx.x;
  if (i >= total) return;
  const int G = dx.C >> 3;
  long r = i / G;
  const int g = (int)(i - r * G);
  const int wb = (int)(r % WB); r /= WB;
  const int hb = (int)(r % HB); r /= HB;
  const int t = (int)(r % dx.T);
  const int b = (int)(r / dx.T);
  const int h0 = 2 * hb, w0 = 2 * wb;
  unsigned long long am[4];
  bool wok[4];
#pragma unroll
  for (int q = 0; q < 4; ++q) {
    const int ho = hb + (q >> 1), wo = wb + (q & 1);
    wok[q] = ho < dy.H && wo < dy.W;
    const long ovox = (((long)b * dy.T + t) * dy.H + (wok[q] ? ho : 0)) * dy.W + (wok[q] ? wo : 0);
    am[q] = wok[q] ? *(const unsigned long long*)(argmax + ovox * dy.C + g * 8) : ~0ull;
  }
  float dv[4][8];
#pragma unroll
  for (int q = 0; q < 4; ++q) {
    bool any = false;
#pragma unroll
    for (int kh = 0; kh < 3; ++kh)
#pragma unroll
      for (int kw = 0; kw < 3; ++kw) {
        const bool in = ((q >> 1) ? kh == 0 : kh >= 1) && ((q & 1) ? kw == 0 : kw >= 1);
        if (!in) continue;
        const unsigned long long x = am[q] ^ ((unsigned long long)(kh * 3 + kw) * 0x0101010101010101ull);
        any |= ((x - 0x0101010101010101ull) & ~x & 0x8080808080808080ull) != 0;
      }
    if (any) ld8<T>((const T*)dy.p + vox_off(dy, b, t, hb + (q >> 1), wb + (q & 1)) + g * 8, dv[q]);
    else {
#pragma unroll
      for (int e = 0; e < 8; ++e) dv[q][e] = 0.f;
    }
  }
#pragma unroll
  for (int ih = 0; ih < 2; ++ih)
#pragma unroll
    for (int iw = 0; iw < 2; ++iw) {
      const int h = h0 + ih, w = w0 + iw;
      if (h >= dx.H || w >= dx.W) continue;
      float gr[8] = {0, 0, 0, 0, 0, 0, 0, 0};
      unsigned long long ex;
      asm volatile("s_mov_b64 %0, exec" : "=s"(ex));
#pragma unroll
      for (int q = 0; q < 4; ++q) {
        const int dh = q >> 1, dw = q & 1;
        const int kh = ih + 1 - 2 * dh, kw = iw + 1 - 2 * dw;
        if (kh < 0 || kw < 0) continue;
        const uint32_t alo = (uint32_t)am[q], ahi = (uint32_t)(am[q] >> 32);
#pragma unroll
        for (int e = 0; e < 8; ++e) POOL_ADD_IF8(gr[e], alo, ahi, e, (uint32_t)(kh * 3 + kw), dv[q][e], ex);
      }
      T* dst = (T*)dx.p + vox_off(dx, b, t, h, w) + g * 8;
      if (accumulate) {
        float o[8];
        ld8<T>(dst, o);
#pragma unroll
        for (int e = 0; e < 8; ++e) gr[e] += o[e];
      }
      st8<T>(dst, gr);
    }
}

template <typename T>
__global__ __launch_bounds__(256) void maxpool_bwd_k3s2_kernel(TView dy, const uint8_t* __restrict__ argmax, TView dx, int accumulate,
                                                               int TB, int HB, int WB, long total) {
  const long i = (long)blockIdx.x * blockDim.x + threadIdx.x;
  if (i >= total) return;
  const int G = dx.C >> 3;
  long r = i / G;
  const int g = (int)(i - r * G);
  const int wb = (int)(r % WB); r /= WB;
  const int hb = (int)(r % HB); r /= HB;
  const int tb = (int)(r % TB);
  const int b = (int)(r / TB);
  unsigned long long am[8];
  float dv[8][8];
#pragma unroll
  for (int w = 0; w < 8; ++w) {
    const int to = tb + (w >> 2), ho = hb + ((w >> 1) & 1), wo = wb + (w & 1);
    const bool ok = to < dy.T && ho < dy.H && wo < dy.W;
    am[w] = ~0ull;
    if (ok) {
      const long ovox = (((long)b * dy.T + to) * dy.H + ho) * dy.W + wo;
      am[w] = *(const unsigned long long*)(argmax + ovox * dy.C + g * 8);
      ld8<T>((const T*)dy.p + vox_off(dy, b, to, ho, wo) + g * 8, dv[w]);
    } else {
#pragma unroll
      for (int e = 0; e < 8; ++e) dv[w][e] = 0.f;
    }
  }
#pragma unroll
  for (int v = 0; v < 8; ++v) {
    const int it = v >> 2, ih = (v >> 1) & 1, iw = v & 1;
    const int t = 2 * tb + it, h = 2 * hb + ih, w_ = 2 * wb + iw;
    if (t >= dx.T || h >= dx.H || w_ >= dx.W) continue;
    float gr[8] = {0, 0, 0, 0, 0, 0, 0, 0};
    unsigned long long ex;
    asm volatile("s_mov_b64 %0, exec" : "=s"(ex));
#pragma unroll
    for (int w = 0; w < 8; ++w) {
      const int dt = w >> 2, dh = (w >> 1) & 1, dw = w & 1;
      if (dt > it || dh > ih || dw > iw) continue;
      const int kt = dt ? 0 : it + 1, kh = dh ? 0 : ih + 1, kw = dw ? 0 : iw + 1;
      const uint32_t alo = (uint32_t)am[w], ahi = (uint32_t)(am[w] >> 32);
#pragma unroll
      for (int e = 0; e < 8; ++e) POOL_ADD_IF8(gr[e], alo, ahi, e, (uint32_t)((kt * 3 + kh) * 3 + kw), dv[w][e], ex);
    }
    T* dst = (T*)dx.p + vox_off(dx, b, t, h, w_) + g * 8;
    if (accumulate) {
      float o[8];
      ld8<T>(dst, o);
#pragma unroll
      for (int e = 0; e < 8; ++e) gr[e] += o[e];
    }
    st8<T>(dst, gr);
  }
}

template <typename T>
__global__ __launch_bounds__(256) void maxpool_bwd_k3s1_twalk_kernel(TView dy, const uint8_t* __restrict__ argmax, TView dx,
                                                                     int accumulate, long total) {
  const long i = (long)blockIdx.x * blockDim.x + threadIdx.x;
  if (i >= total) return;
  const int G = dx.C >> 3;
  const uint32_t col = (uint32_t)(i / G);
  const int g = (int)(i - (long)col * G);
  int b, h, w;
  pool_column(dx, col, b, h, w);
  const int T_ = dx.T, H = dx.H, W = dx.W;
  float g_m[8], g_0[8], g_p[8];
#pragma unroll
  for (int e = 0; e < 8; ++e) { g_m[e] = 0.f; g_0[e] = 0.f; g_p[e] = 0.f; }
  for (int to = 0; to <= T_; ++to) {
    if (to < T_) {
      unsigned long long am[9];
#pragma unroll
      for (int kh = 0; kh < 3; ++kh)
#pragma unroll
        for (int kw = 0; kw < 3; ++kw) {
          const int ho = h + 1 - kh, wo = w + 1 - kw;
          const bool ok = (unsigned)ho < (unsigned)H && (unsigned)wo < (unsigned)W;
          const long ovox = (((long)b * T_ + to) * H + (ok ? ho : 0)) * W + (ok ? wo : 0);
          am[kh * 3 + kw] = ok ? *(const unsigned long long*)(argmax + ovox * dx.C + g * 8) : ~0ull;
        }
#pragma unroll
      for (int kh = 0; kh < 3; ++kh)
#pragma unroll
        for (int kw = 0; kw < 3; ++kw) {
          const unsigned long long s = (unsigned long long)(kh * 3 + kw) * 0x0101010101010101ull;
          const unsigned long long x0 = am[kh * 3 + kw] ^ s, x1 = am[kh * 3 + kw] ^ (s + 9ull * 0x0101010101010101ull),
                                   x2 = am[kh * 3 + kw] ^ (s + 18ull * 0x0101010101010101ull);
          const unsigned long long z0 = (x0 - 0x0101010101010101ull) & ~x0, z1 = (x1 - 0x0101010101010101ull) & ~x1,
                                   z2 = (x2 - 0x0101010101010101ull) & ~x2;
          if (!((z0 | z1 | z2) & 0x8080808080808080ull)) continue;
          float dv[8];
          ld8<T>((const T*)dy.p + vox_off(dy, b, to, h + 1 - kh, w + 1 - kw) + g * 8, dv);
#pragma unroll
          for (int e = 0; e < 8; ++e) {
            if (((x0 >> (8 * e)) & 0xffull) == 0) g_m[e] += dv[e];
            if (((x1 >> (8 * e)) & 0xffull) == 0) g_0[e] += dv[e];
            if (((x2 >> (8 * e)) & 0xffull) == 0) g_p[e] += dv[e];
          }
        }
    }
    const int t = to - 1;
    if (t >= 0) {
      T* dst = (T*)dx.p + vox_off(dx, b, t, h, w) + g * 8;
      if (accumulate) {
        float o[8];
        ld8<T>(dst, o);
#pragma unroll
        for (int e = 0; e < 8; ++e) g_m[e] += o[e];
      }
      st8<T>(dst, g_m);
    }
#pragma unroll
    for (int e = 0; e < 8; ++e) { g_m[e] = g_0[e]; g_0[e] = g_p[e]; g_p[e] = 0.f; }
  }
}

__global__ __launch_bounds__(256) void maxpool_bwd_k3s1_tw3_kernel(TView dy, const uint8_t* __restrict__ argmax, TView dx,
                                                                   int accumulate, long total) {
  const long i = (long)blockIdx.x * blockDim.x + threadIdx.x;
  if (i >= total) return;
  unsigned long long exec0;
  asm volatile("s_mov_b64 %0, exec" : "=s"(exec0));
  const int G = dx.C >> 3;
  const uint32_t col = (uint32_t)(i / G);
  const int g = (int)(i - (long)col * G);
  int b, h, w;
  pool_column(dx, col, b, h, w);
  const int T_ = dx.T, H = dx.H, W = dx.W;
  const uint8_t* amp = argmax + ((((long)b * T_) * H + h) * W + w) * (long)dx.C + g * 8;
  const unsigned short* dyp = (const unsigned short*)dy.p + vox_off(dy, b, 0, h, w) + g * 8;
  const long am_plane = (long)H * W * dx.C, dy_plane = (long)H * W * dy.ld;
  uint32_t okmask = 0;
#pragma unroll
  for (int kh = 0; kh < 3; ++kh)
#pragma unroll
    for (int kw = 0; kw < 3; ++kw) {
      const int ho = h + 1 - kh, wo = w + 1 - kw;
      okmask |= (((unsigned)ho < (unsigned)H && (unsigned)wo < (unsigned)W) ? 1u : 0u) << (kh * 3 + kw);
    }
  float g_m[8], g_0[8], g_p[8];
// ... 201 lines not shown
```

### vinet_amd/engine.py

```python
import ctypes as C
import itertools
import math
import os
import weakref

import torch

from . import _lib as L

F32, BF16 = L.F32, L.BF16
F32S = L.F32S
TORCH_DT = {F32: torch.float32, BF16: torch.bfloat16}
ESIZE = {F32: 4, BF16: 2}
EG = {F32: 4, BF16: 8}

_DEFAULT_DTYPE = BF16
_WEIGHTS_EPOCH = 0
_UNPACK_TABLES = {}
_SIDE_STREAMS = {}

_CONFIG = dict(
    WGRAD_SIDE_STREAM=True,
    WGRAD_CUS=208,
    WGRAD_CUS_DEC=208,
    TAIL_WGRAD_FULL=True,
    WGRAD_GROUP=1,
    WGRAD_GROUP_CAPTURE=16,
    MULTI_UNPACK=1,
    N_SIDE_STREAMS=1,
    BRANCH_STREAMS_VOX=65536,
    BRANCH_STREAMS_EAGER=False,
    BRANCH_STREAMS_TRAIN_VOX=800000,
    BRANCH_STREAMS_TRAIN_BATCH=32,
    BRANCH_STREAMS_BWD=True,
    BRANCH_STREAMS_BWD_MIN_BATCH=8,
    BRANCH_STREAMS_SWAP=True,
    STEM_FOLD=True,
    JOINT_ENTRY=1,
    BN_BWD_FUSE=1,
    SHARE_SKIP_GRAD=True,
    DEFER_DECODER_WGRAD=1,
    DEFER_DECODER_WGRAD_F32S=0,
    PERSISTENT_DW=1,
    MATERIALIZE_NT=800,
    SPLIT_WGRAD_BF16=1,
    SPLIT_IN_APPLY=1,
    DGRAD_BN_STATS=1,
    UPSAMPLE_BWD_RELU=1,
    PARAM_GRAD_MODE="fused",
    DBG_SPIN_SIDE=0,
    DBG_SPIN_MAIN=0,
    DBG_SPIN_FORK=0,
    ABLATE="",
)
globals().update(_CONFIG)
_ABLATE, _ABLATE_TAGS = set(), []


def configure(**kw):
    global _ABLATE, _ABLATE_TAGS
    old = {}
    for k, v in kw.items():
        K = k.upper()
        if K not in _CONFIG:
            raise KeyError("engine.configure: unknown option %r (known: %s)" % (k, ", ".join(sorted(_CONFIG))))
        d = _CONFIG[K]
        if isinstance(d, bool):
            v = (v not in ("0", "false", "False", "")) if isinstance(v, str) else bool(v)
        elif isinstance(d, int):
            v = int(v)
        elif isinstance(d, str):
            v = str(v)
        old[K] = globals()[K]
        globals()[K] = v
        if K == "PARAM_GRAD_MODE":
            set_param_grad_mode(v)
        if K == "ABLATE":
            items = [a for a in v.split(",") if a]
            _ABLATE = set(a for a in items if not a.startswith("tag:"))
            _ABLATE_TAGS = [a[4:] for a in items if a.startswith("tag:")]
            if _ABLATE_TAGS:
                _ABLATE.add("\0tags")
    return old


def configure_from_string(text):
    kw = {}
    for item in filter(None, (text or "").split(",")):
        k, _, v = item.partition("=")
        k = k.strip()
        if k.startswith("lib."):
            L.set_option(k[4:], int(v))
        elif k.upper() == "ABLATE":
            kw["ABLATE"] = v.replace("+", ",")
        else:
            kw[k] = v
    return configure(**kw)


def config(changed_only=False):
    cur = {k: globals()[k] for k in _CONFIG}
    if changed_only:
        cur = {k: v for k, v in cur.items() if v != _CONFIG[k]}
    if L.LIB_OPTIONS:
        cur["lib"] = dict(L.LIB_OPTIONS)
    return cur


def set_default_dtype(name):
    global _DEFAULT_DTYPE
    _DEFAULT_DTYPE = {"bf16": BF16, "bfloat16": BF16, "fp32": F32, "float32": F32, "fp32s": F32S, "fp32_split": F32S}[str(name).replace("torch.", "")]


def default_dtype():
    return _DEFAULT_DTYPE


def bump_weights_epoch():
    global _WEIGHTS_EPOCH
    _WEIGHTS_EPOCH += 1


def rup(a, b):
    return (a + b - 1) // b * b


class Profiler:

    def __init__(self, only=None):
        self.only = None if only is None else set(only)
        self.records = []

    def want(self, key):
        return self.only is None or key in self.only

    def summary(self):
        torch.cuda.synchronize()
        agg = {}
        for key, e0, e1, work in self.records:
            a = agg.setdefault(key, dict(count=0, ms=0.0, work=work))
            a["count"] += 1
            a["ms"] += e0.elapsed_time(e1)
        return agg


PROFILER = None
LAUNCH_LOG = None


def set_profiler(p):
    global PROFILER
    PROFILER = p


def _stream_for(device):
    if device.type == "cuda":
        return torch.cuda.current_stream(device).cuda_stream
    if not L.is_test_double():
        raise RuntimeError("vinet_amd runs on MI355X only: tensor on %s and no HIP device (no CPU fallback)" % device)
    return 0


def _ptr(t):
    return t.data_ptr() if t is not None else None


class View:
    __slots__ = ("buf", "off", "B", "T", "H", "W", "C", "ld", "sB", "dt")

    def __init__(self, buf, off, B, T, H, W, Cc, ld, sB, dt):
        self.buf, self.off, self.B, self.T, self.H, self.W, self.C, self.ld, self.sB, self.dt = buf, off, B, T, H, W, Cc, ld, sB, dt

    @staticmethod
    def alloc(B, T, H, W, Cc, dt, device, zero=False):
        ld = Cc
        n = B * T * H * W * ld
        buf = (torch.zeros if zero else torch.empty)(n, dtype=TORCH_DT[dt], device=device)
        return View(buf, 0, B, T, H, W, Cc, ld, T * H * W * ld, dt)

    @property
    def device(self):
        return self.buf.device

    @property
    def nvox(self):
        return self.B * self.T * self.H * self.W

    def ptr(self):
        return self.buf.data_ptr() + self.off * ESIZE[self.dt]

    def ct(self):
        return L.CTensor(self.ptr(), self.B, self.T, self.H, self.W, self.C, self.ld, self.sB)

    def chan(self, c0, c1):
        assert 0 <= c0 < c1 <= self.C
        return View(self.buf, self.off + c0, self.B, self.T, self.H, self.W, c1 - c0, self.ld, self.sB, self.dt)

    def tslice(self, t0, t1):
        assert 0 <= t0 < t1 <= self.T
        return View(self.buf, self.off + t0 * self.H * self.W * self.ld, self.B, t1 - t0, self.H, self.W, self.C, self.ld, self.sB, self.dt)

    def quads(self):
        assert self.ld == self.C and self.sB == self.T * self.H * self.W * self.C
        n = self.nvox * self.C
        assert n % 4 == 0
        return View(self.buf, self.off, 1, 1, 1, n // 4, 4, 4, n, self.dt)

    def torch5(self):
        return torch.as_strided(self.buf, (self.B, self.T, self.H, self.W, self.C),
                                (self.sB, self.H * self.W * self.ld, self.W * self.ld, self.ld, 1), self.off)

    def same_dims(self, o):
        return (self.B, self.T, self.H, self.W, self.C) == (o.B, o.T, o.H, o.W, o.C)


class Act:
    __slots__ = ("v", "scale", "shift", "relu", "_grad", "grad_ready", "needs_grad", "parent", "pc0", "pt0", "fold",
                 "indep", "ready_of", "grad_marks", "mean", "invstd", "alias_of", "n_readers", "act_out", "grad_masked", "prows")

    def __init__(self, v, scale=None, shift=None, relu=False, needs_grad=False, mean=None, invstd=None):
        self.v, self.scale, self.shift, self.relu = v, scale, shift, relu
        self.mean, self.invstd = mean, invstd
        self._grad, self.grad_ready, self.needs_grad = None, False, needs_grad
        self.parent, self.pc0, self.pt0 = None, 0, 0
        self.fold = None
        self.indep = False
        self.ready_of = None
        self.grad_marks = 0
        self.alias_of = None
        self.n_readers = 0
        self.act_out = 0
        self.grad_masked = -1
        self.prows = None

    @property
    def plain(self):
        return self.scale is None and not self.relu

    def affine(self):
        return L.CAffine(_ptr(self.scale), _ptr(self.shift), 1 if self.relu else 0)

    def sub_chan(self, c0, c1):
        a = Act(self.v.chan(c0, c1), None if self.scale is None else self.scale[c0:c1],
                None if self.shift is None else self.shift[c0:c1], self.relu, self.needs_grad,
                None if self.mean is None else self.mean[c0:c1], None if self.invstd is None else self.invstd[c0:c1])
        a.parent, a.pc0, a.pt0 = self, c0, None
        return a

    def region(self, c0, c1):
        a = self.sub_chan(c0, c1)
        a.indep = True
        return a

    def sub_t(self, t0, t1):
        a = Act(self.v.tslice(t0, t1), self.scale, self.shift, self.relu, self.needs_grad, self.mean, self.invstd)
        a.parent, a.pt0, a.pc0 = self, t0, None
        return a

    def sub_rows(self, r0, thw):
        v, (t, h, w) = self.v, thw
        assert self.plain and v.sB >= v.T * v.H * v.W * v.ld and 0 <= r0 and r0 + t * h * w <= v.T * v.H * v.W
        a = Act(View(v.buf, v.off + r0 * v.ld, v.B, t, h, w, v.C, v.ld, v.sB, v.dt), needs_grad=self.needs_grad)
        a.parent, a.pc0, a.pt0, a.prows = self, None, None, (r0, t, h, w)
        return a

    def root(self):
        a = self
        while a.parent is not None and not a.indep:
            a = a.parent
        return a

    def grad_view(self, dt=None, zero=False):
        if self.parent is not None:
            if self.indep and zero:
                top = self.parent
                while top.parent is not None:
                    top = top.parent
                assert top._grad is None, "zero-filled gradient requested for a region of live shared storage"
            g = self.parent.grad_view(dt, zero)
            if self.prows is not None:
                r0, t, h, w = self.prows
                return View(g.buf, g.off + r0 * g.ld, g.B, t, h, w, g.C, g.ld, g.sB, g.dt)
            if self.pt0 is None:
                return g.chan(self.pc0, self.pc0 + self.v.C)
            return g.tslice(self.pt0, self.pt0 + self.v.T)
        if self._grad is None:
            v = self.v
            self._grad = View.alloc(v.B, v.T, v.H, v.W, v.C, v.dt if dt is None else dt, v.device, zero=zero)
            if zero:
                self.grad_ready = True
        return self._grad

    def is_grad_ready(self):
        if self.ready_of is not None:
            return all(a.is_grad_ready() for a in self.ready_of)
        return self.root().grad_ready

    def mark_grad_ready(self):
        r = self.root()
        r.grad_ready = True
        r.grad_marks += 1


def _abs_chan(a):
    off = 0
    while a.parent is not None:
        if a.pc0 is None:
            return None
        off += a.pc0
        a = a.parent
    return a, off


def _note_reader(ctx, x):
    if ctx.recording and x.needs_grad:
        x.root().n_readers += 1


def _register_bnb(ctx, x, ws, rows):
    loc = _abs_chan(x)
    if loc is None:
        return
    owner, off = loc
    r = x.root()
    ctx._bnb.setdefault(id(owner), []).append((off, off + x.v.C, ws, rows, r, r.grad_marks))


def _find_bnb(ctx, res, c0, width):
    loc = _abs_chan(res)
    if loc is None or id(loc[0]) not in ctx._bnb:
        return None
    owner, off = loc
    a0, a1 = off + c0, off + c0 + width
    for r0, r1, ws, rows, root, marks in reversed(ctx._bnb[id(owner)]):
        if r0 <= a0 and a1 <= r1 and root.grad_marks == marks:
            return ws, rows, a0 - r0, r1 - r0
    return None


class Ctx:

    def __init__(self, device, dt=None, training=False, record=False):
        self.lib = L.get()
        self.device = device
        dt = _DEFAULT_DTYPE if dt is None else dt
        self.dt = F32 if dt == F32S else dt
        self.cdt = dt
        self.training = training
        self.tape = [] if record else None
        self.stream = _stream_for(device)
        self._bnb = {}
        self._side_rr = -1
        self._begin_backward()

    def _begin_backward(self, capturing=False):
        self.capturing = capturing
        self.side_used = False
        self._side_keep = []
        self._deferred = []
        self._unpack_jobs = []
        self._dw_plans = []
        self._joined = False
        self.bwd_cm = None
        self._tape_left = len(self.tape) if self.tape else 0

    @property
    def recording(self):
        return self.tape is not None

    def f32(self, n, zero=False):
        return (torch.zeros if zero else torch.empty)(n, dtype=torch.float32, device=self.device)

    def call(self, name, *args, tag=None, work=None):
        if LAUNCH_LOG is not None:
            LAUNCH_LOG.append((name, args[-1] if args else None, tag))
        if _ABLATE and (name in _ABLATE or (tag is not None and any(a in tag for a in _ABLATE_TAGS))):
            return
        prof = PROFILER
        if prof is not None and self.device.type == "cuda" and prof.want(tag or name):
            e0, e1 = torch.cuda.Event(enable_timing=True), torch.cuda.Event(enable_timing=True)
            e0.record()
            rc = getattr(self.lib, name)(*args)
            e1.record()
            prof.records.append((tag or name, e0, e1, work))
        else:
            rc = getattr(self.lib, name)(*args)
        if rc != 0:
            L.check(rc, name)

    def record(self, fn):
        if self.tape is not None:
            self.tape.append(fn)

    def side_stream(self, k=0):
        if not WGRAD_SIDE_STREAM or self.device.type != "cuda":
            return None
        return self._stream(k)

    def _stream(self, k):
        st = _SIDE_STREAMS.get((self.device.index, k))
        if st is None:
            st = _SIDE_STREAMS[(self.device.index, k)] = torch.cuda.Stream(self.device)
        return st

    def branch_streams(self, nvox, batch=0):
        if self.device.type != "cuda":
            return None
        if self.training or self.recording:
            if nvox > BRANCH_STREAMS_TRAIN_VOX or batch > BRANCH_STREAMS_TRAIN_BATCH:
                return None
        else:
            if nvox > BRANCH_STREAMS_VOX:
                return None
            if not BRANCH_STREAMS_EAGER and not torch.cuda.is_current_stream_capturing():
                return None
        return [self._stream(k) for k in ("b1", "b2")]

    def on_stream(self, st, fork=True):
        return _OnStream(self, st, fork)

    def side_streams(self):
        if self.side_stream() is None:
            return []
        return [self.side_stream(k) for k in range(N_SIDE_STREAMS)]

    def keep(self, *tensors):
        self._side_keep.extend(t for t in tensors if t is not None)

    def flush_deferred(self):
        jobs, self._deferred = self._deferred, []
        if not jobs:
            return
        side = self.side_stream()
        if side is not None:
            cur = torch.cuda.current_stream(self.device)
            for st in self.side_streams():
                st.wait_stream(cur)
            self._joined = True
        try:
            for job in jobs:
                job()
        finally:
            self._joined = False

    def flush_unpack(self):
        jobs, self._unpack_jobs = self._unpack_jobs, []
        if not jobs:
            return
        uniq = {}
        for j in jobs:
            uniq.setdefault(j[0], j)
        key = jobs = tuple(uniq.values())
        ent = _UNPACK_TABLES.get(key)
        if ent is None:
# ... 435 lines not shown
        db = _param_grad(self.beta) if self.beta is not None and self.beta.requires_grad else None
        ctx.call("vinet_bn_bwd_finalize", ws.data_ptr() + (o if ws_off is None else 4 * ws_off), rows, N, ld, float(M), scale.data_ptr() + o, 1 if train_bn else 0,
                 _ptr(dg), _ptr(db), invstd.data_ptr() + o, c1.data_ptr() + o, c2.data_ptr() + o, ctx.stream)
        _note_param_grad(ctx, self.gamma, self.beta)


class JointBN:

    def __init__(self, members, widths, fold_cache=None):
        self.members, self.widths = list(members), list(widths)
        self.offs = [sum(widths[:i]) for i in range(len(widths))]
        self.N = sum(widths)
        self.fold_cache = fold_cache
        self.eps, self.momentum = members[0].eps, members[0].momentum

    def fold_stamp(self, bias, dt, device):
        return tuple(m.fold_stamp(None, dt, device) for m in self.members)

    def fold(self, ctx, bias, N, scale, shift, invstd=None):
        assert bias is None and N == self.N
        for m, w, o in zip(self.members, self.widths, self.offs):
            m.fold(ctx, None, w, scale, shift, invstd, off=o)

    def finalize(self, ctx, stats, rows, N, M, mean, invstd, scale, shift):
        for m, w, o in zip(self.members, self.widths, self.offs):
            m.finalize(ctx, stats, rows, w, M, mean, invstd, scale, shift, off=o, ld=N)

    def bwd_finalize(self, ctx, ws, rows, N, M, scale, train_bn, invstd, c1, c2):
        for m, w, o in zip(self.members, self.widths, self.offs):
            m.bwd_finalize(ctx, ws, rows, w, M, scale, train_bn, invstd, c1, c2, off=o, ld=N)


PARAM_GRAD_HOOK = None


def _note_param_grad(ctx, *params):
    if PARAM_GRAD_HOOK is not None:
        for p in params:
            if p is not None and p.requires_grad:
                PARAM_GRAD_HOOK(ctx, p)


def _param_grad(p):
    if p.grad is None:
        p.grad = torch.zeros_like(p, memory_format=torch.contiguous_format)
    return p.grad


def _kernel_name(ctx, d):
    buf = C.create_string_buffer(96)
    wgrad = isinstance(d, L.CWgradDesc)
    (ctx.lib.vinet_conv3d_wgrad_kernel_name if wgrad else ctx.lib.vinet_conv3d_kernel_name)(C.byref(d), buf, 96)
    return buf.value.decode() or ("wgrad" if wgrad else "conv")


def _splitk_scratch(ctx, d):
    nbytes = ctx.lib.vinet_conv3d_splitk_bytes(C.byref(d))
    if nbytes <= 0:
        return None
    ws = torch.empty(nbytes // 4, dtype=torch.float32, device=ctx.device)
    d.splitk_ws, d.splitk_ws_bytes = ws.data_ptr(), nbytes
    return ws


def _conv_desc(ctx, mode, xv, yv, odims, stride, omul, ooff, ntaps, taps, w, kp, pre, n_valid, promise, accumulate):
    d = L.CConvDesc()
    d.dtype, d.out_dtype, d.mode = ctx.cdt, yv.dt, mode
    d.x, d.y = xv.ct(), yv.ct()
    d.oT, d.oH, d.oW = odims
    d.sT, d.sH, d.sW = stride
    d.omT, d.omH, d.omW = omul
    d.ooT, d.ooH, d.ooW = ooff
    d.ntaps, d.taps, d.w, d.Kp = ntaps, _ptr(taps), w.data_ptr(), kp
    d.pre, d.n_valid, d.accumulate = pre, n_valid, accumulate
    d.tline, d.tpad = promise
    return d


def _set_bnb(d, zv, fwd, mean, invstd, c1=None, c2=None):
    d.bnb_z, d.bnb_ld, d.bnb_sB, d.bnb_fwd = zv.ptr(), zv.ld, zv.sB, fwd
    d.bnb_mean, d.bnb_invstd = mean.data_ptr(), invstd.data_ptr()
    if c1 is not None:
        d.bnb_c1, d.bnb_c2 = c1.data_ptr(), c2.data_ptr()


def _conv_prof(ctx, kernel, kind, plan, xv, M, ex, ey, ew, parts=1, suffix=""):
    tag = None
    if PROFILER is not None:
        tag = (kernel if isinstance(kernel, str) else _kernel_name(ctx, kernel)) + suffix + " | " + kind + " " + plan.site(xv)
    nw = plan.N * plan.Cin * plan.ntaps
    return tag, dict(flops=2.0 * M * nw / parts, bytes=float(xv.nvox * plan.Cin * ex + M * plan.N * ey + nw * ew) / parts)


def _run_conv(ctx, d, out_scale, out_shift, act, stats, tag, work, splitk=False):
    d.out_scale, d.out_shift, d.act, d.stats = out_scale, out_shift, act, stats
    ws = _splitk_scratch(ctx, d) if splitk else None
    ctx.call("vinet_conv3d", C.byref(d), ctx.stream, tag=tag, work=work)


def conv_forward(ctx, plan, x, bn=None, act=L.ACT_NONE, dst=None, out_dt=None, n_pad=None):
    _note_reader(ctx, x)
    want_plain = (MATERIALIZE_NT and x.scale is not None and ctx.dt != L.F32 and x.fold is None and not plan.stem and
                  plan.N * plan.ntaps >= MATERIALIZE_NT and x.v.dt == ctx.dt)
    xv = x.v
    folded = plan.stem and x.fold is not None
    if folded:
        odims = xv.T, (x.fold[0] - 1) // 2 + 1, (x.fold[1] - 1) // 2 + 1
    else:
        odims = plan.out_dims(xv.T, xv.H, xv.W)
    Ny = plan.N if n_pad is None else n_pad
    if dst is None:
        dst = Act(View.alloc(xv.B, odims[0], odims[1], odims[2], Ny, ctx.dt if out_dt is None else out_dt, xv.device))
    out = dst.v
    given = (dst.scale, dst.shift, dst.mean, dst.invstd)
    dst.mean = dst.invstd = None
    assert (out.B, out.T, out.H, out.W, out.C) == (xv.B,) + tuple(odims) + (Ny,), "conv output view mismatch"
    taps, ntaps = plan.folded_taps(ctx.device) if folded else plan.fwd_taps(ctx.device)
    w = plan.packed(ctx, False)
    d = _conv_desc(ctx, L.CONV_STEM if (plan.stem and not folded) else L.CONV_GENERIC, xv, out, odims,
                   (1, 2, 1) if folded else plan.s, (1, 1, 1), (0, 0, 0), ntaps, taps, w, plan.kp(False), x.affine(),
                   plan.N if Ny != plan.N else 0, plan.promise("fwd", folded), 0)
    if want_plain and not ctx.lib.vinet_conv3d_applies_pre_once(C.byref(d)):
        x = materialize(ctx, x)
        xv = x.v
        d.x, d.pre = xv.ct(), x.affine()
    M = xv.B * odims[0] * odims[1] * odims[2]
    es = ESIZE[ctx.dt]
    tag, work = _conv_prof(ctx, d, "fwd", plan, xv, M, es, ESIZE[out.dt], es)

    train_bn = bn is not None and ctx.training
    keep = {}
    res = dst
    res.needs_grad = True
    if bn is None:
        _run_conv(ctx, d, None, _ptr(plan.bias), act, None, tag, work, splitk=True)
        res.scale = res.shift = None
        res.relu = False
        res.act_out = act
    elif train_bn:
        rows = ctx.lib.vinet_conv3d_stats_rows(C.byref(d))
        stats = ctx.f32(rows * 2 * plan.N)
        _run_conv(ctx, d, None, _ptr(plan.bias), L.ACT_NONE, stats.data_ptr(), tag, work)
        scale, shift, mean, invstd = (ctx.f32(plan.N) if g is None else g for g in given)
        if rows >= 1024:
            per = (rows + 255) // 256
            rows2 = (rows + per - 1) // per
            stats2 = ctx.f32(rows2 * 2 * plan.N)
            ctx.call("vinet_bn_partials_fold", stats.data_ptr(), rows, plan.N, stats2.data_ptr(), rows2, ctx.stream)
            stats, rows = stats2, rows2
        bn.finalize(ctx, stats, rows, plan.N, M, mean, invstd, scale, shift)
        res.scale, res.shift, res.relu = scale, shift, (act == L.ACT_RELU)
        keep.update(mean=mean, invstd=invstd)
        res.mean, res.invstd = mean, invstd
    else:
        scale, shift = (ctx.f32(plan.N) if g is None else g for g in given[:2])
        if ctx.recording:
            assert not isinstance(bn, JointBN), "joint convs are not recorded under eval-mode BN"
            invstd = ctx.f32(plan.N)
            bn.fold(ctx, None, plan.N, scale, shift, invstd)
            _run_conv(ctx, d, None, _ptr(plan.bias), L.ACT_NONE, None, tag, work)
            res.scale, res.shift, res.relu = scale, shift, (act == L.ACT_RELU)
            keep.update(mean=bn.rm, invstd=invstd)
        else:
            cached = None
            if given[0] is None and given[1] is None and bn.fold_cache is not None:
                stamp = bn.fold_stamp(plan.bias, ctx.dt, ctx.device)
                cached = bn.fold_cache.get("fold")
                if cached is not None and cached[0] == stamp:
                    scale, shift = cached[1], cached[2]
                else:
                    cached = None
                    bn.fold_cache["fold"] = (stamp, scale, shift)
            if cached is None:
                bn.fold(ctx, plan.bias, plan.N, scale, shift)
            _run_conv(ctx, d, scale.data_ptr(), shift.data_ptr(), act, None, tag, work, splitk=True)
            res.scale = res.shift = None
            res.relu = False

    if ctx.recording:
        ctx.record(lambda: _conv_backward(ctx, plan, x, res, bn, act, train_bn, keep, M))
    return res


class _OnStream:

    def __init__(self, ctx, st, fork):
        self.ctx, self.st, self.fork = ctx, st, fork

    def __enter__(self):
        if self.st is None:
            return self
        self.prev = self.ctx.stream
        self.cm = torch.cuda.stream(self.st)
        self.cm.__enter__()
        self.ctx.stream = self.st.cuda_stream
        if DBG_SPIN_FORK and self.fork and self.ctx.device.type == "cuda" and not torch.cuda.is_current_stream_capturing():
            self.ctx.lib.vinet_debug_spin(abs(DBG_SPIN_FORK), self.st.cuda_stream if DBG_SPIN_FORK > 0 else self.prev)
        return self

    def __exit__(self, *exc):
        if self.st is None:
            return False
        self.ctx.stream = self.prev
        return self.cm.__exit__(*exc)


def _split_planes_folded(ctx, x):
    v = x.v
    B, T, Hp, Wp = v.B, v.T, v.H, 2 * v.W
    n = B * T * Hp * Wp * 4
    src = View(v.buf, v.off, B, T, Hp, Wp, 4, 4, T * Hp * Wp * 4, F32)
    acts = []
    bufs = [torch.empty(n + 64, dtype=TORCH_DT[BF16], device=v.device) for _ in range(2)]
    for b in bufs:
        b[n:].zero_()
    hi, lo = (View(b, 0, B, T, Hp, Wp, 4, 4, T * Hp * Wp * 4, BF16) for b in bufs)
    ctx.call("vinet_split_bf16", C.byref(src.ct()), L.CAffine(None, None, 0), C.byref(hi.ct()), C.byref(lo.ct()), ctx.stream)
    for b in bufs:
        a = Act(View(b, 0, B, T, Hp, Wp // 2, 32, 8, T * Hp * Wp * 4, BF16))
        a.fold = x.fold
        acts.append(a)
    return acts


def _split_planes(ctx, x, dy, dy_planes=None):
    out = []
    if x.fold is not None:
        if dy_planes is None:
            hi = View.alloc(dy.B, dy.T, dy.H, dy.W, dy.C, BF16, dy.device)
            lo = View.alloc(dy.B, dy.T, dy.H, dy.W, dy.C, BF16, dy.device)
            ctx.call("vinet_split_bf16", C.byref(dy.ct()), L.CAffine(None, None, 0), C.byref(hi.ct()), C.byref(lo.ct()), ctx.stream)
            dy_planes = (hi, lo)
        return [tuple(_split_planes_folded(ctx, x)), dy_planes]
    for v, aff in ((x.v, x.affine()),) + (((dy, L.CAffine(None, None, 0)),) if dy_planes is None else ()):
        hi = View.alloc(v.B, v.T, v.H, v.W, v.C, BF16, v.device)
        lo = View.alloc(v.B, v.T, v.H, v.W, v.C, BF16, v.device)
        ctx.call("vinet_split_bf16", C.byref(v.ct()), aff, C.byref(hi.ct()), C.byref(lo.ct()), ctx.stream)
        out.append((hi, lo))
    if dy_planes is not None:
        out.append(dy_planes)
    return out


def _wgrad_desc(ctx, plan, x, dy, dw=None):
    folded = plan.stem and x.fold is not None
    taps, ntaps = plan.folded_taps(ctx.device) if folded else plan.fwd_taps(ctx.device)
    wd = L.CWgradDesc()
    wd.dtype, wd.mode = ctx.cdt, (L.CONV_STEM if (plan.stem and not folded) else L.CONV_GENERIC)
    wd.x, wd.dy = x.v.ct(), dy.ct()
    wd.sT, wd.sH, wd.sW = (1, 2, 1) if folded else plan.s
    wd.ntaps, wd.taps, wd.dw, wd.Kp = ntaps, taps.data_ptr(), (dw.data_ptr() if dw is not None else None), plan.kp(False)
    wd.pre = x.affine()
    wd.tline, wd.tpad = plan.promise("wgrad", folded)
    wd._keep = taps
    return wd


def _conv_backward(ctx, plan, x, res, bn, act, train_bn, keep, M):
    dz = res.grad_view()
    assert res.is_grad_ready(), "conv backward reached before any consumer produced a gradient"
    fused_bnb = dy_planes = None
    if bn is not None:
        dy, fused_bnb, dy_planes = _bn_backward(ctx, plan, x, res, bn, train_bn, keep, M, dz)
    else:
        dy = _act_backward(ctx, res, act, dz)
    if plan.bias is not None and plan.bias.requires_grad:
        _bias_grad(ctx, plan, dy)
    if plan.wants_wgrad():
        for w_ in plan.grad_targets():
            _param_grad(w_)
        _schedule_wgrad(ctx, _WgradJob(ctx, plan, x, dy, M, bn is None, fused_bnb, dy_planes))
    if x.needs_grad:
        _data_grad(ctx, plan, x, res.v, dy, M)


def _bn_backward(ctx, plan, x, res, bn, train_bn, keep, M, dz):
    out, Ny = res.v, res.v.C
    fwd = res.affine()
    mean, invstd = keep["mean"], keep["invstd"]
    nb = float(dz.nvox * dz.C * ESIZE[dz.dt])
    members = list(zip(bn.members, bn.offs, bn.widths)) if isinstance(bn, JointBN) else [(bn, 0, Ny)]
    c1, c2 = ctx.f32(Ny), ctx.f32(Ny)
    left = []
    for m_, o_, w_ in members:
        part = _find_bnb(ctx, res, o_, w_) if DGRAD_BN_STATS else None
        if part is None:
            left.append((m_, o_, w_))
        else:
            m_.bwd_finalize(ctx, part[0], part[1], w_, M, res.scale, train_bn, invstd, c1, c2, off=o_, ld=part[3], ws_off=part[2])
    regions = [(0, Ny, left)] if len(left) == len(members) else [(o_, w_, [(m_, o_, w_)]) for m_, o_, w_ in left]
    for r0, rw, mem in regions:
        dzs, outs = (dz, out) if rw == Ny else (dz.chan(r0, r0 + rw), out.chan(r0, r0 + rw))
        rows = ctx.lib.vinet_stats_rows(C.byref(dzs.ct()))
        ws = ctx.f32(rows * 2 * rw)
        fsl = L.CAffine(res.scale.data_ptr() + 4 * r0, res.shift.data_ptr() + 4 * r0, 1 if res.relu else 0)
        ctx.call("vinet_bn_bwd_reduce", C.byref(dzs.ct()), C.byref(outs.ct()), dz.dt, fsl, mean.data_ptr() + 4 * r0,
                 invstd.data_ptr() + 4 * r0, ws.data_ptr(), ctx.stream, tag=_bn_tag("reduce", rw, dz),
                 work=dict(flops=0.0, bytes=2 * nb * rw / Ny))
        for m_, o_, w_ in mem:
            m_.bwd_finalize(ctx, ws, rows, w_, M, res.scale, train_bn, invstd, c1, c2, off=o_, ld=rw, ws_off=o_ - r0)
    if BN_BWD_FUSE and not x.needs_grad and plan.wants_wgrad() and plan.bias is None and out.dt == dz.dt == ctx.dt:
        fused = (out, fwd, mean, invstd, c1, c2)
        q = _wgrad_desc(ctx, plan, x, dz)
        _set_bnb(q, *fused)
        if ctx.lib.vinet_conv3d_wgrad_fuses_bn_bwd(C.byref(q)):
            return dz, fused, None
    if (SPLIT_IN_APPLY and SPLIT_WGRAD_BF16 and ctx.cdt == F32S and plan.wants_wgrad() and dz.dt == F32 and
            out.dt == F32 and dz.C % 8 == 0 and dz.ld % 8 == 0 and out.ld % 8 == 0 and ctx.device.type == "cuda"):
        dh = View.alloc(dz.B, dz.T, dz.H, dz.W, dz.C, BF16, dz.device)
        dl = View.alloc(dz.B, dz.T, dz.H, dz.W, dz.C, BF16, dz.device)
        ctx.call("vinet_bn_bwd_apply_split", C.byref(dz.ct()), C.byref(out.ct()), fwd, mean.data_ptr(), invstd.data_ptr(),
                 c1.data_ptr(), c2.data_ptr(), C.byref(dz.ct()), C.byref(dh.ct()), C.byref(dl.ct()), ctx.stream,
                 tag=_bn_tag("apply", dz.C, dz), work=dict(flops=0.0, bytes=4 * nb))
        return dz, None, (dh, dl)
    ctx.call("vinet_bn_bwd_apply", C.byref(dz.ct()), C.byref(out.ct()), dz.dt, fwd, mean.data_ptr(), invstd.data_ptr(),
             c1.data_ptr(), c2.data_ptr(), C.byref(dz.ct()), ctx.stream, tag=_bn_tag("apply", dz.C, dz),
             work=dict(flops=0.0, bytes=3 * nb))
    return dz, None, None


def _bn_tag(what, width, dz):
    return ("vinet_bn_bwd_%s | C%d x %d voxels" % (what, width, dz.nvox)) if PROFILER is not None else None


def _act_backward(ctx, res, act, dz):
    if act == L.ACT_RELU and res.grad_masked == res.root().grad_marks and dz.dt == ctx.dt:
        return dz
    if act == L.ACT_NONE and dz.dt == ctx.dt:
        return dz
    dy = dz if dz.dt == ctx.dt else View.alloc(dz.B, dz.T, dz.H, dz.W, dz.C, ctx.dt, dz.device)
    if act != L.ACT_NONE:
        ctx.call("vinet_act_bwd", C.byref(dz.ct()), dz.dt, C.byref(res.v.ct()), res.v.dt, act, C.byref(dy.ct()), dy.dt, ctx.stream)
    else:
        ctx.call("vinet_copy_affine", C.byref(dz.ct()), dz.dt, L.CAffine(None, None, 0), C.byref(dy.ct()), dy.dt, 0, ctx.stream)
    return dy


def _bias_grad(ctx, plan, dy):
    Ny = dy.C
    rows = ctx.lib.vinet_stats_rows(C.byref(dy.ct()))
    ws = ctx.f32(rows * 2 * Ny)
    gb = _param_grad(plan.bias)
    assert Ny % plan.N == 0 and (Ny == plan.N or plan.N == 1)
    ctx.call("vinet_channel_sum", C.byref(dy.ct()), dy.dt, ws.data_ptr(), plan.N, gb.data_ptr(), 1, ctx.stream)
    _note_param_grad(ctx, plan.bias)


class _WgradJob:
    __slots__ = ("ctx", "plan", "x", "dy", "M", "bn_free", "fused_bnb", "dy_planes", "want_planes")

    def __init__(self, ctx, plan, x, dy, M, bn_free, fused_bnb, dy_planes):
        self.ctx, self.plan, self.x, self.dy, self.M, self.bn_free = ctx, plan, x, dy, M, bn_free
        self.fused_bnb, self.dy_planes = fused_bnb, dy_planes
        self.want_planes = bool(SPLIT_WGRAD_BF16 and ctx.cdt == F32S and fused_bnb is None and dy.C % 8 == 0 and x.v.dt == F32 and dy.dt == F32 and
                                ((not plan.stem and x.fold is None and x.v.C % 8 == 0) or
                                 (plan.stem and x.fold is not None and x.scale is None and x.v.off == 0)))

    def __call__(self):
        ctx = self.ctx
        ctx._side_rr = (ctx._side_rr + 1) % N_SIDE_STREAMS
        side = ctx.side_stream(ctx._side_rr)
        if side is not None:
            if not ctx._joined:
                side.wait_stream(torch.cuda.current_stream(ctx.device))
            ctx.side_used = True
        with ctx.on_stream(side, fork=False):
            self._launch(side)
        _note_param_grad(ctx, *self.plan.grad_targets())

    def _launch(self, side):
        ctx, plan, x, dy, M, fused_bnb = self.ctx, self.plan, self.x, self.dy, self.M, self.fused_bnb
        Ny = dy.C
        kp = plan.kp(False)
        nsl = 7 if plan.stem else plan.ntaps
        persistent = bool(PERSISTENT_DW)
        dw = plan.dw_workspace(ctx, nsl * Ny * kp) if persistent else ctx.f32(nsl * Ny * kp, zero=True)
        if persistent:
            ctx._dw_plans.append(plan)
        if persistent and any(j[0] == dw.data_ptr() for j in ctx._unpack_jobs):
            plan.unpack_wgrad(ctx, dw, clear=True)
        wd = _wgrad_desc(ctx, plan, x, dy, dw)
        if fused_bnb is not None:
            _set_bnb(wd, *fused_bnb)
        tail = TAIL_WGRAD_FULL and side is not None and not x.needs_grad and ctx._tape_left <= 1
        wd.max_cus = 256 if (tail or side is None) else (WGRAD_CUS_DEC if self.bn_free else WGRAD_CUS)
        if DBG_SPIN_SIDE and side is not None:
            ctx.lib.vinet_debug_spin(DBG_SPIN_SIDE, ctx.stream)
        if self.want_planes:
            (xh, xl), (dh, dl) = _split_planes(ctx, x, dy, self.dy_planes)
            for xa, da in ((xh, dl), (xl, dh), (xh, dh)):
                wq = _wgrad_desc(ctx, plan, xa if isinstance(xa, Act) else Act(xa), da, dw)
                wq.dtype, wq.max_cus = BF16, wd.max_cus
                tag, work = _conv_prof(ctx, wq, "wgrad(split x3)", plan, x.v, M, 2, 2, 4)
                work["flops"] /= 3
                ctx.call("vinet_conv3d_wgrad", C.byref(wq), ctx.stream, tag=tag, work=work)
            if side is not None:
                ctx.keep(*((p.v if isinstance(p, Act) else p).buf for p in (xh, xl, dh, dl)))
        else:
            tag, work = _conv_prof(ctx, wd, "wgrad", plan, x.v, M, ESIZE[ctx.dt], ESIZE[ctx.dt], 4)
            ctx.call("vinet_conv3d_wgrad", C.byref(wd), ctx.stream, tag=tag, work=work)
        if Ny != plan.N:
            assert plan.ntaps == 1, "channel-padded outputs are only supported for 1x1x1 convs"
        if persistent and MULTI_UNPACK and PARAM_GRAD_HOOK is None and N_SIDE_STREAMS == 1:
            ctx._unpack_jobs.extend(plan.unpack_jobs(dw))
        else:
            plan.unpack_wgrad(ctx, dw, clear=persistent)
        if side is not None:
            ctx.keep(dw, dy.buf, x.v.buf, x.scale, x.shift, *(fused_bnb[2:] if fused_bnb is not None else ()))


def _schedule_wgrad(ctx, job):
    defer = DEFER_DECODER_WGRAD_F32S if ctx.cdt == F32S else DEFER_DECODER_WGRAD
    group = WGRAD_GROUP_CAPTURE if ctx.capturing else WGRAD_GROUP
    if defer and job.bn_free and ctx.side_stream() is not None:
        ctx._deferred.append(job)
    elif group > 1 and ctx.side_stream() is not None:
        ctx._deferred.append(job)
        if len(ctx._deferred) >= group:
            ctx.flush_deferred()
    else:
        ctx.flush_deferred()
        job()


def _bnb_partials(ctx, d, a):
    _set_bnb(d, a.v, a.affine(), a.mean, a.invstd)
    rows = ctx.lib.vinet_conv3d_bn_bwd_stats_rows(C.byref(d))
    if rows <= 0:
        return None
    ws = ctx.f32(rows * 2 * a.v.C)
    d.bnb_partials = ws.data_ptr()
    return ws, rows


def _data_grad(ctx, plan, x, out, dy, M):
    xv = x.v
    if DBG_SPIN_MAIN and ctx.device.type == "cuda":
        ctx.lib.vinet_debug_spin(DBG_SPIN_MAIN, ctx.stream)
    phases, full = plan.dgrad_phases((xv.T, xv.H, xv.W), (out.T, out.H, out.W), ctx.device)
    dx = x.grad_view(zero=not (full or x.is_grad_ready()))
    acc = 1 if x.is_grad_ready() else 0
    wt = plan.packed(ctx, True)
    n_valid = plan.Cin if xv.C != plan.Cin else 0
    es = ESIZE[ctx.dt]
    if plan.temporal and plan.s[0] > 1 and len(phases) > 1:
        d = _conv_desc(ctx, L.CONV_GENERIC, dy, dx, (xv.T, xv.H, xv.W), (plan.s[0], 1, 1), (1, 1, 1), (0, 0, 0), plan.k[0], None,
                       wt, plan.kp(True), L.CAffine(None, None, 0), n_valid, plan.promise("dgrad_fused"), acc)
        if ctx.lib.vinet_conv3d_fuses_dgrad_phases(C.byref(d)):
            part = None
            if (DGRAD_BN_STATS and not acc and x.mean is not None and x.scale is not None and x.parent is None and
                    x.fold is None and xv.dt == dx.dt and xv.C == plan.Cin and dx.same_dims(xv)):
                part = _bnb_partials(ctx, d, x)
            tag, work = _conv_prof(ctx, "conv_tsd_kernel", "dgrad", plan, xv, M, es, es, es)
            ctx.call("vinet_conv3d", C.byref(d), ctx.stream, tag=tag, work=work)
            x.mark_grad_ready()
            if part is not None:
                _register_bnb(ctx, x, *part)
            return
    bx = x.alias_of if x.alias_of is not None else x
    want_bnb = (DGRAD_BN_STATS >= 2 and len(phases) == 1 and full and bx.mean is not None and bx.scale is not None and bx.relu
                and bx.fold is None and ctx.cdt == BF16 and dx.dt == BF16 and bx.v.dt == BF16 and xv.C == plan.Cin
                and dx.same_dims(bx.v) and x.root().grad_marks + 1 == x.root().n_readers)
    part = None
    for ph in phases:
        d = _conv_desc(ctx, L.CONV_GENERIC, dy, dx, ph["Q"], (1, 1, 1), plan.s, ph["r"], ph["ntaps"], ph["taps"], wt, plan.kp(True),
                       L.CAffine(None, None, 0), n_valid, ph["promise"], acc)
        if want_bnb:
            part = _bnb_partials(ctx, d, bx)
        tag, work = _conv_prof(ctx, d, "dgrad", plan, xv, M, es, es, es, len(phases), "+bnb" if part is not None else "")
        ctx.call("vinet_conv3d", C.byref(d), ctx.stream, tag=tag, work=work)
    x.mark_grad_ready()
    if part is not None:
        _register_bnb(ctx, bx, *part)



def maxpool_forward(ctx, x, k, s, p, dst=None):
    xv = x.v
    od = tuple((d + 2 * pp - kk) // ss + 1 for d, kk, ss, pp in zip((xv.T, xv.H, xv.W), k, s, p))
    if dst is None:
        dst = Act(View.alloc(xv.B, od[0], od[1], od[2], xv.C, xv.dt, xv.device))
    out = dst.v
    assert (out.T, out.H, out.W, out.C) == (od[0], od[1], od[2], xv.C) and dst.plain
    pd = L.CPoolDesc(xv.dt, k[0], k[1], k[2], s[0], s[1], s[2], p[0], p[1], p[2])
    rec = ctx.recording and x.needs_grad
    _note_reader(ctx, x)
    am = torch.empty(out.nvox * out.C, dtype=torch.uint8, device=xv.device) if rec else None
    ptag = "maxpool k%dx%dx%d s%dx%dx%d C%d in%dx%dx%dx%d" % (k + s + (xv.C, xv.B, xv.T, xv.H, xv.W))
    es = ESIZE[xv.dt]
    ctx.call("vinet_maxpool3d", C.byref(pd), C.byref(xv.ct()), x.affine(), C.byref(out.ct()), _ptr(am), ctx.stream,
             tag="maxpool_fwd_kernel | " + ptag, work=dict(flops=0.0, bytes=float((xv.nvox + out.nvox) * xv.C * es)))
    dst.needs_grad = x.needs_grad
    if rec:
        def bwd():
            dy = dst.grad_view()
            dx = x.grad_view()
            ctx.call("vinet_maxpool3d_bwd", C.byref(pd), C.byref(dy.ct()), am.data_ptr(), C.byref(dx.ct()),
                     1 if x.is_grad_ready() else 0, ctx.stream, tag="maxpool_bwd_kernel | " + ptag,
                     work=dict(flops=0.0, bytes=float((xv.nvox + out.nvox) * xv.C * es + out.nvox * xv.C)))
            x.mark_grad_ready()
        ctx.record(bwd)
    return dst


def upsample2x_forward(ctx, x, dst=None):
    assert x.plain, "upsample input must be materialised"
    xv = x.v
    if dst is None:
        dst = Act(View.alloc(xv.B, xv.T, 2 * xv.H, 2 * xv.W, xv.C, xv.dt, xv.device))
    out = dst.v
    assert dst.plain
    ctx.call("vinet_upsample2x", C.byref(xv.ct()), C.byref(out.ct()), xv.dt, ctx.stream)
    _note_reader(ctx, x)
    dst.needs_grad = x.needs_grad
    if ctx.recording and x.needs_grad:
        def bwd():
            dy = dst.grad_view()
            dx = x.grad_view()
            if UPSAMPLE_BWD_RELU and x.act_out == L.ACT_RELU and not x.is_grad_ready() and x.parent is None and dx.dt == xv.dt:
                ctx.call("vinet_upsample2x_bwd_relu", C.byref(dy.ct()), C.byref(dx.ct()), C.byref(xv.ct()), dx.dt, ctx.stream)
                x.mark_grad_ready()
                x.grad_masked = x.root().grad_marks
                return
            ctx.call("vinet_upsample2x_bwd", C.byref(dy.ct()), C.byref(dx.ct()), dx.dt, 1 if x.is_grad_ready() else 0, ctx.stream)
            x.mark_grad_ready()
        ctx.record(bwd)
    return dst


def unfold1d_forward(ctx, x, k, stride, pad):
    assert x.plain and not x.needs_grad, "unfold1d: raw input signals only"
    xv = x.v
    assert xv.H == 1 and xv.W == 1
    To = (xv.T + 2 * pad - k) // stride + 1
    dst = Act(View.alloc(xv.B, To, 1, 1, k, xv.dt, xv.device))
    ctx.call("vinet_unfold1d", C.byref(xv.ct()), C.byref(dst.v.ct()), xv.dt, stride, pad, ctx.stream)
    dst.needs_grad = False
    return dst



_PARAM_GRAD_MODE = "fused"


def set_param_grad_mode(mode):
    global _PARAM_GRAD_MODE, PARAM_GRAD_MODE
    assert mode in ("fused", "autograd")
    _PARAM_GRAD_MODE = PARAM_GRAD_MODE = mode


def param_grad_mode():
    return _PARAM_GRAD_MODE


class _TapeFn(torch.autograd.Function):

    @staticmethod
    def forward(fctx, body, n_in, *tensors):
        inputs = tensors[:n_in]
        ectx = body.make_ctx(inputs[0].device, record=True)
        outs, state = body.run(ectx, inputs, [t.requires_grad for t in inputs])
        fctx.body, fctx.ectx, fctx.state, fctx.n_par = body, ectx, state, len(tensors) - n_in
        fctx.params = tensors[n_in:]
        return tuple(outs)

    @staticmethod
    def backward(fctx, *gouts):
        ectx = fctx.ectx
        ectx.stream = _stream_for(ectx.device)
        if _PARAM_GRAD_MODE == "fused":
            gin = fctx.body.seed(ectx, fctx.state, gouts)
            return (None, None) + tuple(gin) + (None,) * fctx.n_par
        params = fctx.params
        saved = [p.grad for p in params]
        for p in params:
            p.grad = None
        try:
            gin = fctx.body.seed(ectx, fctx.state, gouts)
            grads = [p.grad for p in params]
        finally:
            for p, g in zip(params, saved):
                p.grad = g
        base = 2 + len(gin)
        grads = [g if fctx.needs_input_grad[base + i] else None for i, g in enumerate(grads)]
        return (None, None) + tuple(gin) + tuple(grads)


def run_root(body, inputs, params):
    want = torch.is_grad_enabled() and (any(t.requires_grad for t in inputs) or any(p.requires_grad for p in params))
    if want:
        return _TapeFn.apply(body, len(inputs), *inputs, *[p for p in params if p.requires_grad])
    ectx = body.make_ctx(inputs[0].device, record=False)
    outs, _ = body.run(ectx, inputs, [False] * len(inputs))
    return tuple(outs)


class BlockBody:

    def __init__(self, module, fwd, cpad=None):
        self.module, self.fwd, self.cpad = module, fwd, cpad

    def make_ctx(self, device, record):
        return Ctx(device, getattr(self.module, "compute_dtype", None), self.module.training, record)

    def run(self, ectx, inputs, req):
        acts = [import_ncdhw(ectx, t, self.cpad, needs_grad=r) for t, r in zip(inputs, req)]
        outs = self.fwd(ectx, *acts)
        outs = list(outs) if isinstance(outs, (list, tuple)) else [outs]
        for o in outs:
            _note_reader(ectx, o)
        tens = [export_ncdhw(ectx, o, self.out_channels(o)) for o in outs]
        return tens, (acts, outs, [t.shape[1] for t in inputs])

    @staticmethod
    def out_channels(o):
        return o.v.C

    def seed(self, ectx, state, gouts):
        acts, outs, cin = state
        for o, g in zip(outs, gouts):
            import_grad_ncdhw(ectx, o, g)
        ectx.run_backward()
        return [export_grad_ncdhw(ectx, a, c) if (a.needs_grad and a.is_grad_ready()) else None for a, c in zip(acts, cin)]
```

Before: 700.1 clips/s.

## Fuse maxpool backward scatter into BN backward reduce and apply kernels

```diff
diff --git a/include/vinet_hip.h b/include/vinet_hip.h
--- a/include/vinet_hip.h
+++ b/include/vinet_hip.h
@@ -153,6 +153,13 @@
                                 const uint8_t* argmax, char* buf, int32_t n);
 int vinet_maxpool3d_bwd_kernel_name(const VinetPoolDesc* d, const VinetTensor* dy, const uint8_t* argmax,
                                     const VinetTensor* dx, char* buf, int32_t n);
+int vinet_bn_bwd_pool_ok(const VinetPoolDesc* pool, const VinetTensor* z, const VinetTensor* dp, const VinetTensor* dx, int32_t dtype);
+int vinet_bn_bwd_reduce_pool(const VinetPoolDesc* pool, const VinetTensor* dp, const uint8_t* argmax, const VinetTensor* gacc,
+                             int32_t accumulate, const VinetTensor* z, int32_t dtype, VinetAffine fwd, const float* mean,
+                             const float* invstd, float* partials, void* stream);
+int vinet_bn_bwd_apply_pool(const VinetPoolDesc* pool, const VinetTensor* dp, const uint8_t* argmax, const VinetTensor* gacc,
+                            int32_t accumulate, const VinetTensor* z, int32_t dtype, VinetAffine fwd, const float* mean,
+                            const float* invstd, const float* c1, const float* c2, const VinetTensor* dx, void* stream);
 
 int vinet_upsample2x(const VinetTensor* x, const VinetTensor* y, int32_t dtype, void* stream);
 int vinet_upsample2x_bwd(const VinetTensor* dy, const VinetTensor* dx, int32_t dtype, int32_t accumulate, void* stream);
diff --git a/vinet_amd/_lib.py b/vinet_amd/_lib.py
--- a/vinet_amd/_lib.py
+++ b/vinet_amd/_lib.py
@@ -91,6 +91,9 @@
     "vinet_bn_bwd_finalize": [_vp, _i32, _i32, _i32, _f64, _vp, _i32, _vp, _vp, _vp, _vp, _vp, _vp],
     "vinet_bn_bwd_apply": [_PT, _PT, _i32, CAffine, _vp, _vp, _vp, _vp, _PT, _vp],
     "vinet_bn_bwd_apply_split": [_PT, _PT, CAffine, _vp, _vp, _vp, _vp, _PT, _PT, _PT, _vp],
+    "vinet_bn_bwd_pool_ok": [_PP, _PT, _PT, _PT, _i32],
+    "vinet_bn_bwd_reduce_pool": [_PP, _PT, _vp, _PT, _i32, _PT, _i32, CAffine, _vp, _vp, _vp, _vp],
+    "vinet_bn_bwd_apply_pool": [_PP, _PT, _vp, _PT, _i32, _PT, _i32, CAffine, _vp, _vp, _vp, _vp, _PT, _vp],
     "vinet_act_bwd": [_PT, _i32, _PT, _i32, _i32, _PT, _i32, _vp],
     "vinet_channel_sum": [_PT, _i32, _vp, _i32, _vp, _i32, _vp],
     "vinet_maxpool3d": [_PP, _PT, CAffine, _PT, _vp, _vp],
diff --git a/vinet_amd/build.py b/vinet_amd/build.py
--- a/vinet_amd/build.py
+++ b/vinet_amd/build.py
@@ -15,7 +15,8 @@
          "-Wno-unused-result", "-ffp-contract=off"]
 
 
-GUARDED = {"conv_bf16.hip": ("conv_pw_kernel",), "pool.hip": ("maxpool_bwd",), "conv_bnb.hip": ()}
+GUARDED = {"conv_bf16.hip": ("conv_pw_kernel",), "pool.hip": ("maxpool_bwd",), "bn.hip": ("bn_bwd_reduce_pool", "bn_bwd_apply_pool"),
+           "conv_bnb.hip": ()}
 RESOURCES = os.path.join(CSRC, "obj", "kernel_resources.json")
 
 
diff --git a/vinet_amd/csrc/bn.hip b/vinet_amd/csrc/bn.hip
--- a/vinet_amd/csrc/bn.hip
+++ b/vinet_amd/csrc/bn.hip
@@ -1,4 +1,5 @@
 #include "elementwise.h"
+#include "pool_gather.h"
 
 __global__ void bn_finalize_kernel(const float* __restrict__ partials, int rows, int C, int ld, double count,
                                    const float* gamma, const float* beta, float eps, float momentum,
@@ -631,6 +632,254 @@
   return vn_launch_status("bn_bwd_apply8<split>");
 }
 
+
+VN_DEV void bn_pool_windows(const TView& dp, const uint8_t* __restrict__ argmax, int b, int t, int hb, int wb, int g,
+                            unsigned long long am[4], uint4 dv[4]) {
+  bool wok[4];
+  pool_k133s2_codes(dp, argmax, b, t, hb, wb, g, am, wok);
+#pragma unroll
+  for (int q = 0; q < 4; ++q) {
+    const int ho = wok[q] ? hb + (q >> 1) : hb, wo = wok[q] ? wb + (q & 1) : wb;
+    dv[q] = *(const uint4*)((const bf16_t*)dp.p + vox_off(dp, b, t, ho, wo) + g * 8);
+  }
+}
+template <bool ACC>
+VN_DEV void bn_pool_dz(const unsigned long long am[4], const uint4 dv[4], int ih, int iw, const uint4& old, uint32_t dzw[4]) {
+  float gr[8] = {0, 0, 0, 0, 0, 0, 0, 0};
+  unsigned long long ex;
+  asm volatile("s_mov_b64 %0, exec" : "=s"(ex));
+  pool_k133s2_sum_pk(am, dv, ih, iw, ex, gr);
+  if (ACC) {
+    float o[8];
+    unpack16<bf16_t>(old, o);
+#pragma unroll
+    for (int e = 0; e < 8; ++e) gr[e] += o[e];
+  }
+#pragma unroll
+  for (int h = 0; h < 4; ++h) dzw[h] = pack2bf(gr[2 * h], gr[2 * h + 1]);
+}
+
+template <bool ACC>
+__global__ __launch_bounds__(256, 4) void bn_bwd_reduce_pool_kernel(TView x, TView dp, const uint8_t* __restrict__ argmax, TView gacc,
+                                                                    Affine fwd, const float* mean, const float* invstd, FastDiv dWB,
+                                                                    FastDiv dHB, long nblk, long vb, float* __restrict__ partials) {
+  const int G = x.C / 8;
+  const int Gb = G;
+  const int R = 256 / Gb;
+  const int r = threadIdx.x / Gb;
+  const int g0 = threadIdx.x % Gb;
+  __shared__ float red[256 * 16];
+  const long v0 = vb ? (long)blockIdx.x * vb : (long)blockIdx.x * R;
+  long v1 = vb ? v0 + vb : nblk; if (v1 > nblk) v1 = nblk;
+  const long vstep = vb ? (long)R : (long)gridDim.x * R;
+  const bool relu = fwd.relu != 0;
+  const int g = g0;
+  {
+    float s[8], p[8], mu[8], is[8], sc[8], sh[8];
+#pragma unroll
+    for (int e = 0; e < 8; ++e) { s[e] = 0.f; p[e] = 0.f; mu[e] = 0.f; is[e] = 1.f; sc[e] = 1.f; sh[e] = 0.f; }
+    if (r < R) {
+#pragma unroll
+      for (int e = 0; e < 8; ++e) { mu[e] = mean[g * 8 + e]; is[e] = invstd[g * 8 + e]; }
+      if (relu) {
+#pragma unroll
+        for (int e = 0; e < 8; ++e) { sc[e] = fwd.scale ? fwd.scale[g * 8 + e] : 1.f; sh[e] = fwd.shift ? fwd.shift[g * 8 + e] : 0.f; }
+      }
+      for (long v = v0 + r; v < v1; v += vstep) {
+        int b, t, hb, wb;
+        decode_m((int)v, dWB, dHB, x.dT, b, t, hb, wb);
+        const int h0 = 2 * hb, w0 = 2 * wb;
+        unsigned long long am[4];
+        uint4 dv[4];
+        bn_pool_windows(dp, argmax, b, t, hb, wb, g, am, dv);
+#pragma unroll
+        for (int ih = 0; ih < 2; ++ih) {
+          if (h0 + ih >= x.H) continue;
+          const bool in1 = w0 + 1 < x.W;
+          const long vi = (long)(t * x.H + h0 + ih) * x.W + w0;
+          const bf16_t* xp = (const bf16_t*)x.p + (long)b * x.sB + vi * x.ld + g * 8;
+          const bf16_t* op = (const bf16_t*)gacc.p + (long)b * gacc.sB + vi * gacc.ld + g * 8;
+          uint4 xr[2], og[2];
+#pragma unroll
+          for (int iw = 0; iw < 2; ++iw) {
+            xr[iw] = ld16_nt(xp + (in1 ? iw * x.ld : 0));
+            if (ACC) og[iw] = ld16_nt(op + (in1 ? iw * gacc.ld : 0));
+            else og[iw] = make_uint4(0, 0, 0, 0);
+          }
+#pragma unroll
+          for (int iw = 0; iw < 2; ++iw) {
+            if (iw && !in1) continue;
+            uint32_t gw[4];
+            bn_pool_dz<ACC>(am, dv, ih, iw, og[iw], gw);
+            const uint32_t xw[4] = {xr[iw].x, xr[iw].y, xr[iw].z, xr[iw].w};
+#pragma unroll
+            for (int e = 0; e < 8; ++e) {
+              const float xv = __uint_as_float((e & 1) ? (xw[e >> 1] & 0xffff0000u) : (xw[e >> 1] << 16));
+              float gg = __uint_as_float((e & 1) ? (gw[e >> 1] & 0xffff0000u) : (gw[e >> 1] << 16));
+              if (relu && !(fmaf(xv, sc[e], sh[e]) > 0.f)) gg = 0.f;
+              s[e] += gg;
+              p[e] += gg * (xv - mu[e]) * is[e];
+            }
+          }
+        }
+      }
+    }
+    __syncthreads();
+    if (r < R) {
+#pragma unroll
+      for (int e = 0; e < 8; ++e) { red[threadIdx.x * 16 + e] = s[e]; red[threadIdx.x * 16 + 8 + e] = p[e]; }
+    }
+    __syncthreads();
+    if (r == 0) {
+      for (int rr = 1; rr < R; ++rr)
+#pragma unroll
+        for (int e = 0; e < 8; ++e) { s[e] += red[(rr * Gb + g0) * 16 + e]; p[e] += red[(rr * Gb + g0) * 16 + 8 + e]; }
+      float* o = partials + (long)blockIdx.x * 2 * x.C + g * 8;
+      *(float4*)o = make_float4(s[0], s[1], s[2], s[3]);
+      *(float4*)(o + 4) = make_float4(s[4], s[5], s[6], s[7]);
+      *(float4*)(o + x.C) = make_float4(p[0], p[1], p[2], p[3]);
+      *(float4*)(o + x.C + 4) = make_float4(p[4], p[5], p[6], p[7]);
+    }
+  }
+}
+
+template <bool ACC>
+__global__ __launch_bounds__(256, 4) void bn_bwd_apply_pool_kernel(TView x, TView dp, const uint8_t* __restrict__ argmax, TView gacc,
+                                                                   Affine fwd, const float* mean, const float* invstd, const float* c1,
+                                                                   const float* c2, TView dx, FastDiv dWB, FastDiv dHB, long nblk, long vb) {
+  const int G = x.C / 8;
+  const int Gb = G;
+  const int R = 256 / Gb;
+  const int r = threadIdx.x / Gb;
+  const int g0 = threadIdx.x % Gb;
+  if (r >= R) return;
+  const long v0 = (long)blockIdx.x * vb;
+  long v1 = v0 + vb; if (v1 > nblk) v1 = nblk;
+  const bool relu = fwd.relu != 0;
+  const int g = g0;
+  {
+    float A[8], Bc[8], D[8], sh[8];
+#pragma unroll
+    for (int e = 0; e < 8; ++e) {
+      const int c = g * 8 + e;
+      const float sc = fwd.scale[c], k = sc * invstd[c] * c2[c];
+      A[e] = sc; Bc[e] = -k; D[e] = fmaf(k, mean[c], -sc * c1[c]);
+      sh[e] = fwd.shift[c];
+    }
+    for (long v = v0 + r; v < v1; v += R) {
+      int b, t, hb, wb;
+      decode_m((int)v, dWB, dHB, x.dT, b, t, hb, wb);
+      const int h0 = 2 * hb, w0 = 2 * wb;
+      unsigned long long am[4];
+      uint4 dv[4];
+      bn_pool_windows(dp, argmax, b, t, hb, wb, g, am, dv);
+#pragma unroll
+      for (int ih = 0; ih < 2; ++ih) {
+        if (h0 + ih >= x.H) continue;
+        const bool in1 = w0 + 1 < x.W;
+        const long vi = (long)(t * x.H + h0 + ih) * x.W + w0;
+        const bf16_t* xp = (const bf16_t*)x.p + (long)b * x.sB + vi * x.ld + g * 8;
+        const bf16_t* op = (const bf16_t*)gacc.p + (long)b * gacc.sB + vi * gacc.ld + g * 8;
+        bf16_t* yp = (bf16_t*)dx.p + (long)b * dx.sB + vi * dx.ld + g * 8;
+        uint4 xr[2], og[2];
+#pragma unroll
+        for (int iw = 0; iw < 2; ++iw) {
+          xr[iw] = ld16_nt(xp + (in1 ? iw * x.ld : 0));
+          if (ACC) og[iw] = *(const uint4*)(op + (in1 ? iw * gacc.ld : 0));
+          else og[iw] = make_uint4(0, 0, 0, 0);
+        }
+#pragma unroll
+        for (int iw = 0; iw < 2; ++iw) {
+          if (iw && !in1) continue;
+          uint32_t gw[4], ow[4];
+          bn_pool_dz<ACC>(am, dv, ih, iw, og[iw], gw);
+          const uint32_t xw[4] = {xr[iw].x, xr[iw].y, xr[iw].z, xr[iw].w};
+#pragma unroll
+          for (int h = 0; h < 4; ++h) {
+            float o2[2];
+#pragma unroll
+            for (int k2 = 0; k2 < 2; ++k2) {
+              const int e = 2 * h + k2;
+              const float xv = __uint_as_float(k2 ? (xw[h] & 0xffff0000u) : (xw[h] << 16));
+              float gg = __uint_as_float(k2 ? (gw[h] & 0xffff0000u) : (gw[h] << 16));
+              if (relu && !(fmaf(xv, A[e], sh[e]) > 0.f)) gg = 0.f;
+              o2[k2] = fmaf(A[e], gg, fmaf(Bc[e], xv, D[e]));
+            }
+            ow[h] = pack2bf(o2[0], o2[1]);
+          }
+          st16_nt(yp + iw * dx.ld, make_uint4(ow[0], ow[1], ow[2], ow[3]));
+        }
+      }
+    }
+  }
+}
+
+static int bn_bwd_pool_args(const char* who, const VinetPoolDesc* d, const VinetTensor* z, const VinetTensor* dp, const VinetTensor* dx,
+                            int32_t dtype) {
+  VN_CHECK_ARG(d && z && dp && dx, "%s: null argument", who);
+  VN_CHECK_ARG(dtype == VINET_BF16 && d->dtype == VINET_BF16, "%s: bf16 only (dtype %d, pool dtype %d)", who, dtype, d->dtype);
+  VN_CHECK_ARG(d->kT == 1 && d->kH == 3 && d->kW == 3 && d->sT == 1 && d->sH == 2 && d->sW == 2 && d->pT == 0 && d->pH == 1 && d->pW == 1,
+               "%s: pool %dx%dx%d / s(%d,%d,%d) / p(%d,%d,%d) is not the 1x3x3 / s(1,2,2) / p(0,1,1) pool", who, d->kT, d->kH, d->kW,
+               d->sT, d->sH, d->sW, d->pT, d->pH, d->pW);
+  VN_CHECK_ARG(z->C > 0 && z->C % 8 == 0, "%s: C=%d is not a whole number of 8-channel groups", who, z->C);
+  VN_CHECK_ARG(oct_ok(*z) && oct_ok(*dp) && oct_ok(*dx), "%s: views off the 16-byte, 8-channel grid", who);
+  VN_CHECK_ARG(same_dims(*z, *dx), "%s: z and dx differ in their dims", who);
+  VN_CHECK_ARG(dp->B == z->B && dp->C == z->C && dp->T == z->T && dp->H == (z->H - 1) / 2 + 1 && dp->W == (z->W - 1) / 2 + 1,
+               "%s: dp [%d,%d,%d,%d,%d] is not the pooled shape of z [%d,%d,%d,%d,%d]", who, dp->B, dp->T, dp->H, dp->W, dp->C, z->B,
+               z->T, z->H, z->W, z->C);
+  VN_CHECK_ARG(z->C <= 2048, "%s: C=%d is more than the 256 groups of one workgroup", who, z->C);
+  VN_CHECK_ARG(view_voxels(*z) < (1L << 31), "%s: too many voxels for 32-bit block indices", who);
+  return 0;
+}
+extern "C" int vinet_bn_bwd_pool_ok(const VinetPoolDesc* pool, const VinetTensor* z, const VinetTensor* dp, const VinetTensor* dx,
+                                    int32_t dtype) {
+  return bn_bwd_pool_args("bn_bwd_pool_ok", pool, z, dp, dx, dtype) == 0 ? 1 : 0;
+}
+
+extern "C" int vinet_bn_bwd_reduce_pool(const VinetPoolDesc* pool, const VinetTensor* dp, const uint8_t* argmax, const VinetTensor* gacc,
+                                        int32_t accumulate, const VinetTensor* z, int32_t dtype, VinetAffine fwd, const float* mean,
+                                        const float* invstd, float* partials, void* stream) {
+  VN_CHECK_ARG(gacc || !accumulate, "bn_bwd_reduce_pool: null argument");
+  if (bn_bwd_pool_args("bn_bwd_reduce_pool", pool, z, dp, gacc ? gacc : z, dtype)) return -1;
+  VN_CHECK_ARG(argmax && ((uintptr_t)argmax % 8) == 0 && mean && invstd && partials, "bn_bwd_reduce_pool: null or misaligned argument");
+  VN_CHECK_ARG((fwd.scale != nullptr) == (fwd.shift != nullptr), "bn_bwd_reduce_pool: a forward affine needs both its scale and its shift");
+  const int HB = (z->H + 1) / 2, WB = (z->W + 1) / 2;
+  const long nblk = (long)z->B * z->T * HB * WB;
+  const int rows = stats_rows_for(view_voxels(*z));
+  const long vb = g_vinet_opt_reduce_il ? 0 : (nblk + rows - 1) / rows;
+  const TView zv = make_view(*z), gv = make_view(accumulate ? *gacc : *z);
+  if (accumulate)
+    hipLaunchKernelGGL(bn_bwd_reduce_pool_kernel<true>, dim3(rows), dim3(256), 0, (hipStream_t)stream, zv, make_view(*dp), argmax, gv,
+                       make_affine(fwd), mean, invstd, make_fastdiv((uint32_t)WB), make_fastdiv((uint32_t)HB), nblk, vb, partials);
+  else
+    hipLaunchKernelGGL(bn_bwd_reduce_pool_kernel<false>, dim3(rows), dim3(256), 0, (hipStream_t)stream, zv, make_view(*dp), argmax, gv,
+                       make_affine(fwd), mean, invstd, make_fastdiv((uint32_t)WB), make_fastdiv((uint32_t)HB), nblk, vb, partials);
+  return vn_launch_status("bn_bwd_reduce_pool");
+}
+
+extern "C" int vinet_bn_bwd_apply_pool(const VinetPoolDesc* pool, const VinetTensor* dp, const uint8_t* argmax, const VinetTensor* gacc,
+                                       int32_t accumulate, const VinetTensor* z, int32_t dtype, VinetAffine fwd, const float* mean,
+                                       const float* invstd, const float* c1, const float* c2, const VinetTensor* dx, void* stream) {
+  if (bn_bwd_pool_args("bn_bwd_apply_pool", pool, z, dp, dx, dtype)) return -1;
+  if (accumulate && bn_bwd_pool_args("bn_bwd_apply_pool", pool, z, dp, gacc, dtype)) return -1;
+  VN_CHECK_ARG(argmax && ((uintptr_t)argmax % 8) == 0 && fwd.scale && fwd.shift && mean && invstd && c1 && c2,
+               "bn_bwd_apply_pool: null or misaligned argument");
+  const int HB = (z->H + 1) / 2, WB = (z->W + 1) / 2;
+  const long nblk = (long)z->B * z->T * HB * WB;
+  const int G = z->C / 8, R = 256 / G;
+  long vb = R * 4;
+  while ((nblk + vb - 1) / vb > 16384) vb *= 2;
+  const dim3 grid((unsigned)((nblk + vb - 1) / vb));
+  const TView zv = make_view(*z), gv = make_view(accumulate ? *gacc : *dx);
+  if (accumulate)
+    hipLaunchKernelGGL(bn_bwd_apply_pool_kernel<true>, grid, dim3(256), 0, (hipStream_t)stream, zv, make_view(*dp), argmax, gv,
+                       make_affine(fwd), mean, invstd, c1, c2, make_view(*dx), make_fastdiv((uint32_t)WB), make_fastdiv((uint32_t)HB), nblk, vb);
+  else
+    hipLaunchKernelGGL(bn_bwd_apply_pool_kernel<false>, grid, dim3(256), 0, (hipStream_t)stream, zv, make_view(*dp), argmax, gv,
+                       make_affine(fwd), mean, invstd, c1, c2, make_view(*dx), make_fastdiv((uint32_t)WB), make_fastdiv((uint32_t)HB), nblk, vb);
+  return vn_launch_status("bn_bwd_apply_pool");
+}
+
 template <typename TG, typename TZ, typename TO>
 __global__ void act_bwd_kernel(TView dz, TView z, int act, TView dy, long total) {
   const long i = (long)blockIdx.x * blockDim.x + threadIdx.x;
diff --git a/vinet_amd/csrc/pool.hip b/vinet_amd/csrc/pool.hip
--- a/vinet_amd/csrc/pool.hip
+++ b/vinet_amd/csrc/pool.hip
@@ -1,4 +1,4 @@
-#include "elementwise.h"
+#include "pool_gather.h"
 
 struct PoolP { int kT, kH, kW, sT, sH, sW, pT, pH, pW; FastDiv dsT, dsH, dsW; };
 static inline PoolP make_poolp(const VinetPoolDesc* d) {
@@ -508,21 +508,6 @@
     }
   }
 }
-
-#define POOL_ADD_IF_X(g, word, BYTE, code, v, exec0)                                                                                  \
-  asm volatile("v_cmpx_eq_u32_sdwa vcc, %1, %2 src0_sel:BYTE_" #BYTE " src1_sel:DWORD\n\tv_add_f32_e32 %0, %0, %3\n\ts_mov_b64 exec, %4" \
-               : "+v"(g) : "v"(word), "s"(code), "v"(v), "s"(exec0) : "vcc")
-#define POOL_ADD_IF(g, word, BYTE, code, v) POOL_ADD_IF_X(g, word, BYTE, code, v, exec0)
-#define POOL_ADD_IF8(g, lo, hi, e, code, v, ex)                                           \
-  do {                                                                                      \
-    const uint32_t w_ = (e) < 4 ? (lo) : (hi);                                              \
-    switch ((e) & 3) {                                                                      \
-      case 0: POOL_ADD_IF_X(g, w_, 0, code, v, ex); break;                                  \
-      case 1: POOL_ADD_IF_X(g, w_, 1, code, v, ex); break;                                  \
-      case 2: POOL_ADD_IF_X(g, w_, 2, code, v, ex); break;                                  \
-      default: POOL_ADD_IF_X(g, w_, 3, code, v, ex); break;                                 \
-    }                                                                                       \
-  } while (0)
 
 template <typename T>
 __global__ void maxpool_bwd_kernel(PoolP p, TView dy, const uint8_t* __restrict__ argmax, TView dx, int accumulate,
@@ -680,27 +665,11 @@
   const int h0 = 2 * hb, w0 = 2 * wb;
   unsigned long long am[4];
   bool wok[4];
+  pool_k133s2_codes(dy, argmax, b, t, hb, wb, g, am, wok);
+  float dv[4][8];
 #pragma unroll
   for (int q = 0; q < 4; ++q) {
-    const int ho = hb + (q >> 1), wo = wb + (q & 1);
-    wok[q] = ho < dy.H && wo < dy.W;
-    const long ovox = (((long)b * dy.T + t) * dy.H + (wok[q] ? ho : 0)) * dy.W + (wok[q] ? wo : 0);
-    am[q] = wok[q] ? *(const unsigned long long*)(argmax + ovox * dy.C + g * 8) : ~0ull;
-  }
-  float dv[4][8];
-#pragma unroll
-  for (int q = 0; q < 4; ++q) {
-    bool any = false;
-#pragma unroll
-    for (int kh = 0; kh < 3; ++kh)
-#pragma unroll
-      for (int kw = 0; kw < 3; ++kw) {
-        const bool in = ((q >> 1) ? kh == 0 : kh >= 1) && ((q & 1) ? kw == 0 : kw >= 1);
-        if (!in) continue;
-        const unsigned long long x = am[q] ^ ((unsigned long long)(kh * 3 + kw) * 0x0101010101010101ull);
-        any |= ((x - 0x0101010101010101ull) & ~x & 0x8080808080808080ull) != 0;
-      }
-    if (any) ld8<T>((const T*)dy.p + vox_off(dy, b, t, hb + (q >> 1), wb + (q & 1)) + g * 8, dv[q]);
+    if (pool_k133s2_any(am[q], q)) ld8<T>((const T*)dy.p + vox_off(dy, b, t, hb + (q >> 1), wb + (q & 1)) + g * 8, dv[q]);
     else {
 #pragma unroll
       for (int e = 0; e < 8; ++e) dv[q][e] = 0.f;
@@ -715,15 +684,7 @@
       float gr[8] = {0, 0, 0, 0, 0, 0, 0, 0};
       unsigned long long ex;
       asm volatile("s_mov_b64 %0, exec" : "=s"(ex));
-#pragma unroll
-      for (int q = 0; q < 4; ++q) {
-        const int dh = q >> 1, dw = q & 1;
-        const int kh = ih + 1 - 2 * dh, kw = iw + 1 - 2 * dw;
-        if (kh < 0 || kw < 0) continue;
-        const uint32_t alo = (uint32_t)am[q], ahi = (uint32_t)(am[q] >> 32);
-#pragma unroll
-        for (int e = 0; e < 8; ++e) POOL_ADD_IF8(gr[e], alo, ahi, e, (uint32_t)(kh * 3 + kw), dv[q][e], ex);
-      }
+      pool_k133s2_sum(am, dv, ih, iw, ex, gr);
       T* dst = (T*)dx.p + vox_off(dx, b, t, h, w) + g * 8;
       if (accumulate) {
         float o[8];
diff --git a/vinet_amd/csrc/pool_gather.h b/vinet_amd/csrc/pool_gather.h
--- /dev/null
+++ b/vinet_amd/csrc/pool_gather.h
@@ -0,0 +1,87 @@
+#pragma once
+#include "elementwise.h"
+
+#define POOL_ADD_IF_X(g, word, BYTE, code, v, exec0)                                                                                  \
+  asm volatile("v_cmpx_eq_u32_sdwa vcc, %1, %2 src0_sel:BYTE_" #BYTE " src1_sel:DWORD\n\tv_add_f32_e32 %0, %0, %3\n\ts_mov_b64 exec, %4" \
+               : "+v"(g) : "v"(word), "s"(code), "v"(v), "s"(exec0) : "vcc")
+#define POOL_ADD_IF(g, word, BYTE, code, v) POOL_ADD_IF_X(g, word, BYTE, code, v, exec0)
+#define POOL_ADD_IF8(g, lo, hi, e, code, v, ex)                                           \
+  do {                                                                                      \
+    const uint32_t w_ = (e) < 4 ? (lo) : (hi);                                              \
+    switch ((e) & 3) {                                                                      \
+      case 0: POOL_ADD_IF_X(g, w_, 0, code, v, ex); break;                                  \
+      case 1: POOL_ADD_IF_X(g, w_, 1, code, v, ex); break;                                  \
+      case 2: POOL_ADD_IF_X(g, w_, 2, code, v, ex); break;                                  \
+      default: POOL_ADD_IF_X(g, w_, 3, code, v, ex); break;                                 \
+    }                                                                                       \
+  } while (0)
+
+#define POOL_ADD_IF_PK_X(g, word, BYTE, code, pair, WIDEN, exec0)                                                          \
+  do {                                                                                                                     \
+    float t_;                                                                                                              \
+    asm volatile("v_cmpx_eq_u32_sdwa vcc, %2, %3 src0_sel:BYTE_" #BYTE " src1_sel:DWORD\n\t" WIDEN                         \
+                 "\n\tv_add_f32_e32 %0, %0, %1\n\ts_mov_b64 exec, %5"                                                      \
+                 : "+v"(g), "=&v"(t_) : "v"(word), "s"(code), "v"(pair), "s"(exec0) : "vcc");                              \
+  } while (0)
+#define POOL_WIDEN_LO "v_lshlrev_b32_e32 %1, 16, %4"
+#define POOL_WIDEN_HI "v_and_b32_e32 %1, 0xffff0000, %4"
+#define POOL_ADD_IF8_PK(g, lo, hi, e, code, pair, ex)                                                  \
+  do {                                                                                                 \
+    const uint32_t w_ = (e) < 4 ? (lo) : (hi);                                                         \
+    switch ((e) & 3) {                                                                                 \
+      case 0: POOL_ADD_IF_PK_X(g, w_, 0, code, pair, POOL_WIDEN_LO, ex); break;                        \
+      case 1: POOL_ADD_IF_PK_X(g, w_, 1, code, pair, POOL_WIDEN_HI, ex); break;                        \
+      case 2: POOL_ADD_IF_PK_X(g, w_, 2, code, pair, POOL_WIDEN_LO, ex); break;                        \
+      default: POOL_ADD_IF_PK_X(g, w_, 3, code, pair, POOL_WIDEN_HI, ex); break;                       \
+    }                                                                                                  \
+  } while (0)
+
+
+VN_DEV void pool_k133s2_codes(const TView& dy, const uint8_t* __restrict__ argmax, int b, int t, int hb, int wb, int g,
+                              unsigned long long am[4], bool wok[4]) {
+#pragma unroll
+  for (int q = 0; q < 4; ++q) {
+    const int ho = hb + (q >> 1), wo = wb + (q & 1);
+    wok[q] = ho < dy.H && wo < dy.W;
+    const long ovox = (((long)b * dy.T + t) * dy.H + (wok[q] ? ho : 0)) * dy.W + (wok[q] ? wo : 0);
+    am[q] = wok[q] ? *(const unsigned long long*)(argmax + ovox * dy.C + g * 8) : ~0ull;
+  }
+}
+
+VN_DEV bool pool_k133s2_any(unsigned long long amq, int q) {
+  bool any = false;
+#pragma unroll
+  for (int kh = 0; kh < 3; ++kh)
+#pragma unroll
+    for (int kw = 0; kw < 3; ++kw) {
+      const bool in = ((q >> 1) ? kh == 0 : kh >= 1) && ((q & 1) ? kw == 0 : kw >= 1);
+      if (!in) continue;
+      const unsigned long long x = amq ^ ((unsigned long long)(kh * 3 + kw) * 0x0101010101010101ull);
+      any |= ((x - 0x0101010101010101ull) & ~x & 0x8080808080808080ull) != 0;
+    }
+  return any;
+}
+
+VN_DEV void pool_k133s2_sum(const unsigned long long am[4], const float dv[4][8], int ih, int iw, unsigned long long ex, float gr[8]) {
+#pragma unroll
+  for (int q = 0; q < 4; ++q) {
+    const int dh = q >> 1, dw = q & 1;
+    const int kh = ih + 1 - 2 * dh, kw = iw + 1 - 2 * dw;
+    if (kh < 0 || kw < 0) continue;
+    const uint32_t alo = (uint32_t)am[q], ahi = (uint32_t)(am[q] >> 32);
+#pragma unroll
+    for (int e = 0; e < 8; ++e) POOL_ADD_IF8(gr[e], alo, ahi, e, (uint32_t)(kh * 3 + kw), dv[q][e], ex);
+  }
+}
+VN_DEV void pool_k133s2_sum_pk(const unsigned long long am[4], const uint4 dr[4], int ih, int iw, unsigned long long ex, float gr[8]) {
+#pragma unroll
+  for (int q = 0; q < 4; ++q) {
+    const int dh = q >> 1, dw = q & 1;
+    const int kh = ih + 1 - 2 * dh, kw = iw + 1 - 2 * dw;
+    if (kh < 0 || kw < 0) continue;
+    const uint32_t alo = (uint32_t)am[q], ahi = (uint32_t)(am[q] >> 32);
+    const uint32_t pw[4] = {dr[q].x, dr[q].y, dr[q].z, dr[q].w};
+#pragma unroll
+    for (int e = 0; e < 8; ++e) POOL_ADD_IF8_PK(gr[e], alo, ahi, e, (uint32_t)(kh * 3 + kw), pw[e >> 1], ex);
+  }
+}
diff --git a/vinet_amd/engine.py b/vinet_amd/engine.py
--- a/vinet_amd/engine.py
+++ b/vinet_amd/engine.py
@@ -47,6 +47,7 @@
     SPLIT_IN_APPLY=1,
     DGRAD_BN_STATS=1,
     UPSAMPLE_BWD_RELU=1,
+    POOL_BWD_IN_BN=1,
     PARAM_GRAD_MODE="fused",
     DBG_SPIN_SIDE=0,
     DBG_SPIN_MAIN=0,
@@ -216,7 +217,8 @@
 
 class Act:
     __slots__ = ("v", "scale", "shift", "relu", "_grad", "grad_ready", "needs_grad", "parent", "pc0", "pt0", "fold",
-                 "indep", "ready_of", "grad_marks", "mean", "invstd", "alias_of", "n_readers", "act_out", "grad_masked", "prows")
+                 "indep", "ready_of", "grad_marks", "mean", "invstd", "alias_of", "n_readers", "act_out", "grad_masked", "prows", "bn1",
+                 "pool_rec")
 
     def __init__(self, v, scale=None, shift=None, relu=False, needs_grad=False, mean=None, invstd=None):
         self.v, self.scale, self.shift, self.relu = v, scale, shift, relu
@@ -232,6 +234,8 @@
         self.act_out = 0
         self.grad_masked = -1
         self.prows = None
+        self.bn1 = False
+        self.pool_rec = None
 
     @property
     def plain(self):
@@ -284,6 +288,8 @@
             if self.pt0 is None:
                 return g.chan(self.pc0, self.pc0 + self.v.C)
             return g.tslice(self.pt0, self.pt0 + self.v.T)
+        if self.pool_rec is not None:
+            self.pool_rec.flush(self)
         if self._grad is None:
             v = self.v
             self._grad = View.alloc(v.B, v.T, v.H, v.W, v.C, v.dt if dt is None else dt, v.device, zero=zero)
@@ -300,6 +306,32 @@
         r = self.root()
         r.grad_ready = True
         r.grad_marks += 1
+
+
+class _PoolRec:
+    __slots__ = ("x", "pd", "dp", "am", "acc", "launch")
+
+    def __init__(self, x, pd, dp, am, acc, launch):
+        self.x, self.pd, self.dp, self.am, self.acc, self.launch = x, pd, dp, am, acc, launch
+
+    def flush(self, owner):
+        owner.pool_rec = None
+        self.launch(self.acc)
+
+
+def _grad_owner(a):
+    while a.parent is not None:
+        a = a.parent
+    return a
+
+
+def _take_pool_rec(res, bn, train_bn, x):
+    owner = _grad_owner(res)
+    rec = owner.pool_rec
+    if rec is None or rec.x is not res or bn is None or isinstance(bn, JointBN) or not train_bn or not x.needs_grad:
+        return None
+    owner.pool_rec = None
+    return rec
 
 
 def _abs_chan(a):
@@ -1041,6 +1073,7 @@
         res.scale, res.shift, res.relu = scale, shift, (act == L.ACT_RELU)
         keep.update(mean=mean, invstd=invstd)
         res.mean, res.invstd = mean, invstd
+        res.bn1 = not isinstance(bn, JointBN)
     else:
         scale, shift = (ctx.f32(plan.N) if g is None else g for g in given[:2])
         if ctx.recording:
@@ -1146,11 +1179,12 @@
 
 
 def _conv_backward(ctx, plan, x, res, bn, act, train_bn, keep, M):
+    pool = _take_pool_rec(res, bn, train_bn, x)
     dz = res.grad_view()
     assert res.is_grad_ready(), "conv backward reached before any consumer produced a gradient"
     fused_bnb = dy_planes = None
     if bn is not None:
-        dy, fused_bnb, dy_planes = _bn_backward(ctx, plan, x, res, bn, train_bn, keep, M, dz)
+        dy, fused_bnb, dy_planes = _bn_backward(ctx, plan, x, res, bn, train_bn, keep, M, dz, pool)
     else:
         dy = _act_backward(ctx, res, act, dz)
     if plan.bias is not None and plan.bias.requires_grad:
@@ -1163,11 +1197,24 @@
         _data_grad(ctx, plan, x, res.v, dy, M)
 
 
-def _bn_backward(ctx, plan, x, res, bn, train_bn, keep, M, dz):
+def _bn_backward(ctx, plan, x, res, bn, train_bn, keep, M, dz, pool=None):
     out, Ny = res.v, res.v.C
     fwd = res.affine()
     mean, invstd = keep["mean"], keep["invstd"]
     nb = float(dz.nvox * dz.C * ESIZE[dz.dt])
+    if pool is not None:
+        nq = float(pool.dp.nvox * dz.C)
+        rows = ctx.lib.vinet_stats_rows(C.byref(out.ct()))
+        ws = ctx.f32(rows * 2 * Ny)
+        c1, c2 = ctx.f32(Ny), ctx.f32(Ny)
+        ctx.call("vinet_bn_bwd_reduce_pool", C.byref(pool.pd), C.byref(pool.dp.ct()), pool.am.data_ptr(), C.byref(dz.ct()), pool.acc,
+                 C.byref(out.ct()), dz.dt, fwd, mean.data_ptr(), invstd.data_ptr(), ws.data_ptr(), ctx.stream,
+                 tag=_bn_tag("reduce", Ny, dz, " pool"), work=dict(flops=0.0, bytes=(1 + pool.acc) * nb + 3 * nq))
+        bn.bwd_finalize(ctx, ws, rows, Ny, M, res.scale, train_bn, invstd, c1, c2, off=0, ld=Ny, ws_off=0)
+        ctx.call("vinet_bn_bwd_apply_pool", C.byref(pool.pd), C.byref(pool.dp.ct()), pool.am.data_ptr(), C.byref(dz.ct()), pool.acc,
+                 C.byref(out.ct()), dz.dt, fwd, mean.data_ptr(), invstd.data_ptr(), c1.data_ptr(), c2.data_ptr(), C.byref(dz.ct()),
+                 ctx.stream, tag=_bn_tag("apply", Ny, dz, " pool"), work=dict(flops=0.0, bytes=(2 + pool.acc) * nb + 3 * nq))
+        return dz, None, None
     members = list(zip(bn.members, bn.offs, bn.widths)) if isinstance(bn, JointBN) else [(bn, 0, Ny)]
     c1, c2 = ctx.f32(Ny), ctx.f32(Ny)
     left = []
@@ -1208,8 +1255,8 @@
     return dz, None, None
 
 
-def _bn_tag(what, width, dz):
-    return ("vinet_bn_bwd_%s | C%d x %d voxels" % (what, width, dz.nvox)) if PROFILER is not None else None
+def _bn_tag(what, width, dz, mark=""):
+    return ("vinet_bn_bwd_%s | C%d x %d voxels%s" % (what, width, dz.nvox, mark)) if PROFILER is not None else None
 
 
 def _act_backward(ctx, res, act, dz):
@@ -1381,15 +1428,40 @@
              tag="maxpool_fwd_kernel | " + ptag, work=dict(flops=0.0, bytes=float((xv.nvox + out.nvox) * xv.C * es)))
     dst.needs_grad = x.needs_grad
     if rec:
-        def bwd():
+        def launch(acc):
             dy = dst.grad_view()
             dx = x.grad_view()
             ctx.call("vinet_maxpool3d_bwd", C.byref(pd), C.byref(dy.ct()), am.data_ptr(), C.byref(dx.ct()),
-                     1 if x.is_grad_ready() else 0, ctx.stream, tag="maxpool_bwd_kernel | " + ptag,
+                     acc, ctx.stream, tag="maxpool_bwd_kernel | " + ptag,
                      work=dict(flops=0.0, bytes=float((xv.nvox + out.nvox) * xv.C * es + out.nvox * xv.C)))
+
+        def bwd():
+            acc = 1 if x.is_grad_ready() else 0
+            if _pool_bwd_defers(ctx, x, pd, k, s, p):
+                dy, dx = dst.grad_view(), x.grad_view()
+                if dy.dt == dx.dt == BF16 and ctx.lib.vinet_bn_bwd_pool_ok(C.byref(pd), C.byref(xv.ct()), C.byref(dy.ct()),
+                                                                          C.byref(dx.ct()), xv.dt):
+                    _grad_owner(x).pool_rec = _PoolRec(x, pd, dy, am, acc, launch)
+                    x.mark_grad_ready()
+                    return
+            launch(acc)
             x.mark_grad_ready()
         ctx.record(bwd)
     return dst
+
+
+def _pool_bwd_defers(ctx, x, pd, k, s, p):
+    if not (POOL_BWD_IN_BN and x.bn1 and x.relu and x.scale is not None and x.mean is not None and x.fold is None and x.prows is None
+            and x.alias_of is None and ctx.cdt == BF16 and x.v.dt == BF16 and (k, s, p) == ((1, 3, 3), (1, 2, 2), (0, 1, 1))
+            and getattr(ctx.lib, "vinet_bn_bwd_pool_ok", None) is not None and hasattr(ctx.lib, "vinet_bn_bwd_reduce_pool")
+            and hasattr(ctx.lib, "vinet_bn_bwd_apply_pool")):
+        return False
+    r = x.root()
+    if r is x:
+        return x.parent is None and r.grad_marks + 1 == r.n_readers
+    if x.indep or x.pc0 != 0 or x.pt0 is not None or x.parent.v.C != x.v.C:
+        return False
+    return r.grad_marks + 1 == r.n_readers + x.n_readers - 1
 
 
 def upsample2x_forward(ctx, x, dst=None):
```

Measured after the change: 711.9 clips/s, median of 6. +1.7%, better.
